# Alisah-Ozcan/HEonGPU

Hardware: AMD Instinct MI355X
Metric: homomorphic mults/sec (CKKS N=2^16, L=16) + NTT GB/s vs HBM roofline (higher is better)
Workload: dtype u64

## Files before the change

### heongpu_amd/__init__.py

```python
from . import _lib
from .api import (BFV, CKKS, SEC_NONE, SEC_128, SEC_192, SEC_256, TABLES_QP, TABLES_Q_BSK, OP_CKKS_RELIN, OP_CKKS_RESCALE,
                  OP_CKKS_GALOIS, OP_CKKS_ROTATE_HOISTED, OP_BFV_MULTIPLY, OP_BFV_RELIN, OP_BFV_GALOIS, E_INVALID, E_LOGIC, E_RUNTIME,
                  E_NODEVICE, Context, HEError, Rng, TfheContext, OP_KEYGEN_SECRET, OP_KEYGEN_PUBLIC,
                  OP_KEYGEN_SWITCH, OP_CKKS_ENCRYPT, OP_BFV_ENCRYPT, OP_BFV_DECRYPT, OP_BFV_DECODE, OP_CKKS_ENCODE,
                  OP_CKKS_DECODE, OP_BFV_MULTIPLY_PLAIN, OP_MPC_KEY_SHARE, OP_MPC_BFV_DECRYPT_MERGE, OP_MPC_REFRESH_SHARE, OP_MPC_REFRESH_MERGE,
                  MPC_PUBLIC_KEY,
                  MPC_GALOIS_KEY, MPC_RELIN_ROUND1, GATE_NAND, GATE_AND, GATE_AND_FIRST_NOT,
                  GATE_NOR, GATE_OR, GATE_XNOR, GATE_XOR, GATE_NOT, steps_to_galois_elt, linear_transform_plan, encoding_transform_factors, poly_eval_plan, eval_mod_plan, PolyEvalPlan, bootstrap_plan, BootstrapPlan, OP_CKKS_MOD_RAISE, OP_CKKS_BOOTSTRAP, MONOMIAL, CHEBYSHEV, POLY_POWER, POLY_LEAF, POLY_COMBINE, POLY_TAIL_NONE, POLY_TAIL_ONE, to_device, to_host, default_options, broadcast_key, broadcast_bytes, broadcast_path_name,
                  BCAST_FLAT, BCAST_TREE, BCAST_STAGED, BCAST_SAME_DEVICE, OP_CKKS_LOGIC_GATE, OP_BFV_LOGIC_GATE, LOGIC_AND,
                  LOGIC_OR, LOGIC_XOR, LOGIC_NAND, LOGIC_NOR, LOGIC_XNOR, LOGIC_NOT, GATE_B_NONE, GATE_B_CIPHER, GATE_B_PLAIN)

_lib.load()

__all__ = ["BFV", "CKKS", "SEC_NONE", "SEC_128", "SEC_192", "SEC_256", "TABLES_QP", "TABLES_Q_BSK", "Context", "HEError", "Rng",
           "steps_to_galois_elt", "linear_transform_plan", "encoding_transform_factors", "poly_eval_plan", "eval_mod_plan", "PolyEvalPlan", "bootstrap_plan", "BootstrapPlan", "MONOMIAL", "CHEBYSHEV", "POLY_POWER", "POLY_LEAF", "POLY_COMBINE", "POLY_TAIL_NONE", "POLY_TAIL_ONE", "to_device", "to_host", "default_options", "broadcast_key", "broadcast_bytes", "broadcast_path_name",
           "BCAST_FLAT", "BCAST_TREE", "BCAST_STAGED", "BCAST_SAME_DEVICE"]
```

### heongpu_amd/_lib.py

```python
import ctypes
import os

_HERE = os.path.dirname(os.path.abspath(__file__))
LIB_PATH = os.path.join(_HERE, "lib", "libhegpu.so")
if os.environ.get("HEGPU_AUDIT_LIB"):
    if os.path.basename(os.environ["HEGPU_AUDIT_LIB"]) != "libhegpu_audit.so":
        raise ImportError("HEGPU_AUDIT_LIB must name tests/audit/lib/libhegpu_audit.so")
    LIB_PATH = os.environ["HEGPU_AUDIT_LIB"]

u64 = ctypes.c_uint64
u64p = ctypes.c_void_p
c_int = ctypes.c_int
c_size_t = ctypes.c_size_t
voidp = ctypes.c_void_p



class LinearFactor(ctypes.Structure):
    _fields_ = [("diags", ctypes.c_void_p), ("n_diag", c_int), ("index", ctypes.POINTER(c_int)), ("n1", c_int), ("n2", c_int),
                ("baby_keys", ctypes.POINTER(ctypes.c_void_p)), ("baby_elts", ctypes.POINTER(c_int)),
                ("giant_keys", ctypes.POINTER(ctypes.c_void_p)), ("giant_elts", ctypes.POINTER(c_int))]


class PolyStep(ctypes.Structure):
    _fields_ = [("kind", ctypes.c_int32), ("dst", ctypes.c_int32), ("a", ctypes.c_int32), ("b", ctypes.c_int32),
                ("c", ctypes.c_int32), ("level", ctypes.c_int32), ("mul_level", ctypes.c_int32),
                ("rescale_first", ctypes.c_int32), ("rescale_after", ctypes.c_int32), ("n_terms", ctypes.c_int32),
                ("term_reg", ctypes.c_int32 * 15), ("scale", ctypes.c_double), ("tail_const", ctypes.c_double),
                ("w0", ctypes.c_double * 2), ("w", (ctypes.c_double * 2) * 15)]


class BootstrapConfig(ctypes.Structure):
    _fields_ = [("scale", ctypes.c_double), ("message_ratio", ctypes.c_double), ("K", ctypes.c_int32),
                ("sine_degree", ctypes.c_int32), ("double_angle", ctypes.c_int32), ("cts_level", ctypes.c_int32),
                ("cts_pieces", ctypes.c_int32), ("eval_level", ctypes.c_int32), ("stc_level", ctypes.c_int32),
                ("stc_pieces", ctypes.c_int32)]


class BootstrapPlan(ctypes.Structure):
    _fields_ = [("k1", ctypes.c_uint64), ("cts_level", ctypes.c_int32), ("cts_pieces", ctypes.c_int32),
                ("eval_level", ctypes.c_int32), ("stc_level", ctypes.c_int32), ("stc_pieces", ctypes.c_int32),
                ("out_level", ctypes.c_int32), ("K", ctypes.c_int32), ("sine_degree", ctypes.c_int32),
                ("double_angle", ctypes.c_int32), ("reserved", ctypes.c_int32), ("raise_scale", ctypes.c_double),
                ("cts_scale", ctypes.c_double * 5), ("cts_label", ctypes.c_double * 5), ("eval_in_scale", ctypes.c_double),
                ("eval_target_scale", ctypes.c_double), ("eval_out_scale", ctypes.c_double), ("stc_in_scale", ctypes.c_double),
                ("stc_scale", ctypes.c_double * 5), ("stc_label", ctypes.c_double * 5), ("out_scale", ctypes.c_double)]


SIGNATURES = [
    ("hegpu_last_error", ctypes.c_char_p, []),
    ("hegpu_version", ctypes.c_char_p, []),
    ("hegpu_context_create", c_int,
     [c_int, c_int, ctypes.POINTER(c_int), c_int, ctypes.POINTER(c_int), c_int, u64, c_int,
      ctypes.POINTER(voidp)]),
    ("hegpu_context_create_default", c_int, [c_int, c_int, c_int, u64, c_int, ctypes.POINTER(voidp)]),
    ("hegpu_context_create_from_primes", c_int,
     [c_int, c_int, ctypes.POINTER(u64), c_int, c_int, u64, ctypes.POINTER(voidp)]),
    ("hegpu_validate_coeff_modulus_values", c_int, [c_int, ctypes.POINTER(u64), c_int, c_int, c_int]),
    ("hegpu_context_destroy", None, [voidp]),
    ("hegpu_context_upload", c_int, [voidp]),
    ("hegpu_context_clone", c_int, [voidp, ctypes.POINTER(voidp)]),
    ("hegpu_context_upload_device", c_int, [voidp, c_int]),
    ("hegpu_context_device", c_int, [voidp]),
    ("hegpu_broadcast_key", c_int, [ctypes.POINTER(voidp), c_int, ctypes.POINTER(voidp), c_size_t, ctypes.POINTER(voidp)]),
    ("hegpu_broadcast_bytes", c_int, [ctypes.POINTER(c_int), c_int, ctypes.POINTER(voidp), c_size_t, ctypes.POINTER(voidp),
                                      ctypes.POINTER(c_int)]),
    ("hegpu_last_broadcast_path", c_int, []),
    ("hegpu_context_set_option", c_int, [voidp, ctypes.c_char_p, c_int]),
    ("hegpu_context_get_option", c_int, [voidp, ctypes.c_char_p, ctypes.POINTER(c_int)]),
    ("hegpu_tfhe_context_set_option", c_int, [voidp, ctypes.c_char_p, c_int]),
    ("hegpu_context_int", ctypes.c_long, [voidp, ctypes.c_char_p]),
    ("hegpu_context_get", ctypes.c_long, [voidp, ctypes.c_char_p, voidp, ctypes.c_long]),
    ("hegpu_context_device_ptr", voidp, [voidp, ctypes.c_char_p]),
    ("hegpu_steps_to_galois_elt", c_int, [c_int, c_int, c_int]),
    ("hegpu_ntt", c_int, [voidp, c_int, u64p, u64p, c_int, c_int, c_int, c_int, voidp, voidp, voidp]),
    ("hegpu_GPU_NTT", c_int, [voidp, c_int, u64p, u64p, c_int, c_int, c_int, voidp]),
    ("hegpu_GPU_NTT_Inplace", c_int, [voidp, c_int, u64p, c_int, c_int, c_int, voidp]),
    ("hegpu_GPU_INTT", c_int, [voidp, c_int, u64p, u64p, c_int, c_int, c_int, voidp]),
    ("hegpu_GPU_INTT_Inplace", c_int, [voidp, c_int, u64p, c_int, c_int, c_int, voidp]),
    ("hegpu_GPU_NTT_Modulus_Ordered_Inplace", c_int, [voidp, c_int, u64p, c_int, c_int, c_int, c_int, voidp, voidp]),
    ("hegpu_GPU_NTT_Poly_Ordered_Inplace", c_int, [voidp, c_int, u64p, c_int, c_int, c_int, c_int, voidp, voidp]),
    ("hegpu_addition", c_int, [voidp, u64p, u64p, u64p, c_int, c_int, c_int, c_int, voidp]),
    ("hegpu_cross_multiplication", c_int,
     [voidp, c_int, u64p, u64, u64p, u64, u64p, u64, c_int, c_int, voidp]),
    ("hegpu_cipher_broadcast", c_int, [voidp, u64p, u64, u64p, u64, c_int, c_int, c_int, c_int, c_int, voidp]),
    ("hegpu_mod_raise", c_int, [voidp, u64p, u64, u64p, u64, c_int, c_int, c_int, voidp]),
    ("hegpu_ckks_mod_raise", c_int, [voidp, u64p, u64, u64p, u64, c_int, c_int, voidp, c_size_t, voidp]),
    ("hegpu_keyswitch_multiply_accumulate", c_int,
     [voidp, u64p, u64, u64p, u64p, u64, c_int, c_int, c_int, c_int, c_int, c_int, voidp]),
    ("hegpu_base_conversion_DtoQtilde", c_int, [voidp, u64p, u64, u64p, u64, c_int, c_int, voidp]),
    ("hegpu_divide_round_lastq", c_int, [voidp, u64p, u64, u64p, u64, u64p, u64, c_int, c_int, voidp]),
    ("hegpu_divide_round_lastq_permute", c_int,
     [voidp, u64p, u64, u64p, u64, u64p, u64, c_int, c_int, c_int, voidp]),
    ("hegpu_divide_round_lastq_leveled_stage_one", c_int, [voidp, u64p, u64, u64p, u64, c_int, c_int, c_int, voidp]),
    ("hegpu_divide_round_lastq_leveled_stage_two", c_int,
     [voidp, u64p, u64, u64p, u64, u64p, u64, u64p, u64, c_int, c_int, c_int, voidp]),
    ("hegpu_move_cipher_leveled", c_int, [voidp, u64p, u64, u64p, u64, c_int, c_int, voidp]),
    ("hegpu_divide_round_lastq_rescale", c_int, [voidp, u64p, u64, u64p, u64, u64p, u64, c_int, c_int, voidp]),
    ("hegpu_divide_round_lastq_extended", c_int,
     [voidp, u64p, u64, u64p, u64, u64p, u64, c_int, c_int, c_int, voidp]),
    ("hegpu_fast_convertion", c_int, [voidp, u64p, u64, u64p, u64, u64p, u64, c_int, voidp]),
    ("hegpu_fast_floor", c_int, [voidp, u64p, u64, u64p, u64, c_int, voidp]),
    ("hegpu_workspace_bytes", c_size_t, [voidp, c_int, c_int, c_int]),
    ("hegpu_ckks_multiply", c_int, [voidp, u64p, u64, u64p, u64, u64p, u64, c_int, c_int, voidp]),
    ("hegpu_ckks_relinearize_inplace", c_int, [voidp, u64p, u64, u64p, c_int, c_int, voidp, c_size_t, voidp]),
    ("hegpu_probe_ckks_relinearize", c_int,
     [voidp, u64p, u64, u64p, c_int, c_int, voidp, c_size_t, ctypes.c_uint, voidp]),
    ("hegpu_ckks_rescale_inplace", c_int, [voidp, u64p, u64, c_int, c_int, voidp, c_size_t, voidp]),
    ("hegpu_ckks_apply_galois", c_int,
     [voidp, u64p, u64, u64p, u64, u64p, c_int, c_int, c_int, voidp, c_size_t, voidp]),
    ("hegpu_ckks_rotate_hoisted", c_int,
     [voidp, u64p, u64, u64p, u64, ctypes.POINTER(ctypes.c_void_p), ctypes.POINTER(c_int), c_int, c_int, c_int, voidp,
      c_size_t, voidp]),
    ("hegpu_ckks_diag_mac", c_int,
     [voidp, u64p, u64, c_int, u64p, c_int, ctypes.POINTER(c_int), c_int, u64p, u64, c_int, c_int, voidp]),
    ("hegpu_ckks_linear_transform_workspace_bytes", c_size_t, [voidp, c_int, c_int, c_int, c_int]),
    ("hegpu_ckks_linear_transform", c_int,
     [voidp, u64p, u64, u64p, u64, u64p, c_int, ctypes.POINTER(c_int), c_int, c_int, ctypes.POINTER(ctypes.c_void_p),
      ctypes.POINTER(c_int), ctypes.POINTER(ctypes.c_void_p), ctypes.POINTER(c_int), c_int, c_int, voidp, c_size_t, voidp]),
    ("hegpu_encoding_transform_shape", c_int,
     [c_int, c_int, c_int, ctypes.POINTER(c_int), ctypes.POINTER(c_int), ctypes.POINTER(c_int)]),
    ("hegpu_encoding_transform_fill", c_int, [c_int, c_int, c_int, c_int, c_int, ctypes.POINTER(c_int), voidp]),
    ("hegpu_poly_eval_plan_size", c_int,
     [c_int, voidp, c_int, c_int, c_int, c_int, ctypes.c_double, ctypes.c_double, ctypes.POINTER(u64), c_int,
      ctypes.POINTER(c_int)]),
    ("hegpu_poly_eval_plan_fill", c_int,
     [c_int, voidp, c_int, c_int, c_int, c_int, ctypes.c_double, ctypes.c_double, ctypes.POINTER(u64), c_int,
      ctypes.POINTER(PolyStep), c_int]),
    ("hegpu_eval_mod_plan_size", c_int,
     [c_int, c_int, c_int, c_int, ctypes.c_double, ctypes.c_double, ctypes.POINTER(u64), c_int, ctypes.POINTER(c_int)]),
    ("hegpu_eval_mod_plan_fill", c_int,
     [c_int, c_int, c_int, c_int, ctypes.c_double, ctypes.c_double, ctypes.POINTER(u64), c_int, ctypes.POINTER(PolyStep),
      c_int]),
    ("hegpu_ckks_weighted_sum", c_int,
     [voidp, ctypes.POINTER(ctypes.c_void_p), ctypes.POINTER(u64), ctypes.POINTER(c_int), ctypes.POINTER(ctypes.c_double),
      c_int, ctypes.c_double, ctypes.c_double, u64p, u64, c_int, c_int, voidp]),
    ("hegpu_ckks_double_sub", c_int,
     [voidp, u64p, u64, c_int, u64p, u64, c_int, ctypes.c_double, u64p, u64, c_int, c_int, voidp]),
    ("hegpu_ckks_poly_eval_workspace_bytes", c_size_t, [voidp, ctypes.POINTER(PolyStep), c_int, c_int, c_int]),
    ("hegpu_ckks_poly_eval", c_int,
     [voidp, u64p, u64, u64p, u64, ctypes.POINTER(PolyStep), c_int, u64p, c_int, c_int, voidp, c_size_t, voidp]),
    ("hegpu_ckks_conj_split", c_int, [voidp, u64p, u64, u64p, u64, u64p, u64p, u64, c_int, c_int, c_int, voidp]),
    ("hegpu_ckks_conj_merge", c_int, [voidp, u64p, u64, u64p, u64, u64p, u64, c_int, c_int, c_int, voidp]),
    ("hegpu_ckks_encoding_transform_workspace_bytes", c_size_t, [voidp, ctypes.POINTER(LinearFactor), c_int, c_int, c_int]),
    ("hegpu_ckks_coeff_to_slot", c_int,
     [voidp, u64p, u64, u64p, u64p, u64, ctypes.POINTER(LinearFactor), c_int, u64p, c_int, c_int, voidp, c_size_t, voidp]),
    ("hegpu_ckks_slot_to_coeff", c_int,
     [voidp, u64p, u64, u64p, u64, u64p, u64, ctypes.POINTER(LinearFactor), c_int, c_int, c_int, voidp, c_size_t, voidp]),
    ("hegpu_bootstrap_plan_fill", c_int,
     [ctypes.POINTER(BootstrapConfig), ctypes.POINTER(u64), c_int, ctypes.POINTER(BootstrapPlan)]),
    ("hegpu_ckks_bootstrap_workspace_bytes", c_size_t,
     [voidp, ctypes.POINTER(BootstrapPlan), ctypes.POINTER(PolyStep), c_int, ctypes.POINTER(LinearFactor), c_int,
      ctypes.POINTER(LinearFactor), c_int, c_int, c_int]),
    ("hegpu_ckks_bootstrap", c_int,
     [voidp, u64p, u64, u64p, u64, ctypes.POINTER(BootstrapPlan), ctypes.POINTER(PolyStep), c_int,
      ctypes.POINTER(LinearFactor), c_int, ctypes.POINTER(LinearFactor), c_int, u64p, u64p, u64p, u64p, c_int, voidp,
      c_size_t, voidp]),
    ("hegpu_ckks_gate_combine", c_int,
     [voidp, c_int, u64p, u64, c_int, u64p, c_int, u64, c_int, u64p, u64, c_int, ctypes.c_double, u64p, u64, c_int, c_int,
      voidp]),
    ("hegpu_bfv_gate_combine", c_int, [voidp, c_int, u64p, u64, u64p, c_int, u64, u64p, u64, u64p, u64, c_int, voidp]),
    ("hegpu_ckks_logic_gate", c_int,
     [voidp, c_int, u64p, u64, u64p, c_int, u64, u64p, ctypes.c_double, u64p, u64, c_int, c_int, voidp, c_size_t, voidp]),
    ("hegpu_bfv_logic_gate", c_int,
     [voidp, c_int, u64p, u64, u64p, c_int, u64, u64p, u64p, u64, c_int, voidp, c_size_t, voidp]),
    ("hegpu_bfv_multiply", c_int, [voidp, u64p, u64, u64p, u64, u64p, u64, c_int, voidp, c_size_t, voidp]),
    ("hegpu_bfv_relinearize_inplace", c_int, [voidp, u64p, u64, u64p, c_int, voidp, c_size_t, voidp]),
    ("hegpu_bfv_apply_galois", c_int,
     [voidp, u64p, u64, u64p, u64, u64p, c_int, c_int, voidp, c_size_t, voidp]),
    ("hegpu_rng_create", c_int, [u64, ctypes.POINTER(voidp)]),
    ("hegpu_rng_create_seeded", c_int, [ctypes.c_char_p, ctypes.POINTER(voidp)]),
    ("hegpu_rng_create_from_entropy", c_int, [ctypes.POINTER(voidp)]),
    ("hegpu_drbg_block", c_int, [ctypes.c_char_p, u64, u64, ctypes.POINTER(ctypes.c_uint32)]),
    ("hegpu_rng_destroy", None, [voidp]),
    ("hegpu_generate_secret_key", c_int, [voidp, voidp, c_int, u64p, voidp, c_size_t, voidp]),
    ("hegpu_generate_public_key", c_int, [voidp, voidp, u64p, u64p, voidp, c_size_t, voidp]),
    ("hegpu_generate_relin_key", c_int, [voidp, voidp, u64p, u64p, voidp, c_size_t, voidp]),
    ("hegpu_generate_switch_key", c_int, [voidp, voidp, u64p, u64p, u64p, voidp, c_size_t, voidp]),
    ("hegpu_generate_galois_key", c_int, [voidp, voidp, u64p, c_int, u64p, voidp, c_size_t, voidp]),
    ("hegpu_ckks_encrypt", c_int, [voidp, voidp, u64p, u64p, u64p, voidp, c_size_t, voidp]),
    ("hegpu_ckks_decrypt", c_int, [voidp, u64p, u64p, c_int, u64p, voidp]),
    ("hegpu_bfv_encrypt", c_int, [voidp, voidp, u64p, u64p, u64p, voidp, c_size_t, voidp]),
    ("hegpu_bfv_decrypt", c_int, [voidp, u64p, u64p, u64p, voidp, c_size_t, voidp]),
    ("hegpu_mpc_public_key_share", c_int, [voidp, voidp, voidp, u64p, u64p, voidp, c_size_t, voidp]),
    ("hegpu_mpc_relin_key_share_round1", c_int, [voidp, voidp, voidp, u64p, u64p, u64p, voidp, c_size_t, voidp]),
    ("hegpu_mpc_relin_key_share_round2", c_int, [voidp, voidp, u64p, u64p, u64p, u64p, voidp, c_size_t, voidp]),
    ("hegpu_mpc_galois_key_share", c_int, [voidp, voidp, voidp, u64p, c_int, u64p, voidp, c_size_t, voidp]),
    ("hegpu_mpc_accumulate", c_int, [voidp, ctypes.POINTER(ctypes.c_void_p), c_int, c_int, u64p, voidp]),
    ("hegpu_mpc_relin_key_finish", c_int, [voidp, ctypes.POINTER(ctypes.c_void_p), c_int, u64p, u64p, voidp]),
    ("hegpu_mpc_ckks_decrypt_share", c_int, [voidp, voidp, u64p, u64, u64p, c_int, u64p, c_int, voidp]),
    ("hegpu_mpc_ckks_decrypt_merge", c_int,
     [voidp, u64p, u64, ctypes.POINTER(ctypes.c_void_p), c_int, c_int, u64p, c_int, voidp]),
    ("hegpu_mpc_bfv_decrypt_share", c_int, [voidp, voidp, u64p, u64, u64p, u64p, c_int, voidp]),
    ("hegpu_mpc_bfv_decrypt_merge", c_int,
     [voidp, u64p, u64, ctypes.POINTER(ctypes.c_void_p), c_int, u64p, c_int, voidp, c_size_t, voidp]),
    ("hegpu_mpc_ckks_refresh_share", c_int,
     [voidp, voidp, voidp, u64p, u64, u64p, c_int, c_int, u64p, c_int, voidp, c_size_t, voidp]),
    ("hegpu_mpc_ckks_refresh_merge", c_int,
     [voidp, voidp, u64p, u64, ctypes.POINTER(ctypes.c_void_p), c_int, c_int, u64p, u64, c_int, voidp, c_size_t, voidp]),
    ("hegpu_mpc_bfv_refresh_share", c_int, [voidp, voidp, voidp, u64p, u64, u64p, u64p, c_int, voidp, c_size_t, voidp]),
    ("hegpu_mpc_bfv_refresh_merge", c_int,
     [voidp, voidp, u64p, u64, ctypes.POINTER(ctypes.c_void_p), c_int, u64p, u64, c_int, voidp, c_size_t, voidp]),
    ("hegpu_bfv_noise_rns", c_int, [voidp, u64p, u64p, u64p, voidp]),
    ("hegpu_bfv_plain_to_ntt", c_int, [voidp, u64p, u64p, voidp]),
    ("hegpu_negacyclic_shift", c_int, [voidp, u64p, u64p, c_int, c_int, c_int, voidp]),
    ("hegpu_ckks_constant_op", c_int, [voidp, c_int, u64p, ctypes.c_double, u64p, c_int, c_int, voidp]),
    ("hegpu_ckks_gaussian_integer_op", c_int,
     [voidp, c_int, u64p, ctypes.c_double, ctypes.c_double, u64p, c_int, c_int, voidp]),
    ("hegpu_ckks_mult_i", c_int, [voidp, u64p, u64p, c_int, c_int, c_int, voidp]),
    ("hegpu_cipherplain_multiplication", c_int, [voidp, u64p, u64p, u64p, c_int, voidp]),
    ("hegpu_bfv_plain_addsub", c_int, [voidp, u64p, u64p, u64p, c_int, voidp]),
    ("hegpu_bfv_multiply_plain", c_int, [voidp, u64p, u64p, u64p, voidp, c_size_t, voidp]),
    ("hegpu_bfv_encode", c_int, [voidp, voidp, c_int, u64p, voidp]),
    ("hegpu_ckks_encode", c_int, [voidp, voidp, c_int, ctypes.c_double, u64p, voidp, c_size_t, voidp]),
    ("hegpu_ckks_decode", c_int, [voidp, u64p, c_int, ctypes.c_double, voidp, voidp, c_size_t, voidp]),
    ("hegpu_ckks_encode_complex", c_int, [voidp, voidp, c_int, ctypes.c_double, u64p, voidp, c_size_t, voidp]),
    ("hegpu_ckks_decode_complex", c_int, [voidp, u64p, c_int, ctypes.c_double, voidp, voidp, c_size_t, voidp]),
    ("hegpu_ckks_encode_coeff", c_int, [voidp, voidp, c_int, ctypes.c_double, u64p, voidp]),
    ("hegpu_ckks_decode_coeff", c_int, [voidp, u64p, c_int, ctypes.c_double, voidp, voidp, c_size_t, voidp]),
    ("hegpu_ckks_encode_scalar", c_int, [voidp, ctypes.c_double, ctypes.c_double, u64p, voidp]),
    ("hegpu_bfv_decode", c_int, [voidp, u64p, u64p, voidp, c_size_t, voidp]),
    ("hegpu_tfhe_context_create", c_int, [ctypes.POINTER(voidp)]),
    ("hegpu_tfhe_context_destroy", None, [voidp]),
    ("hegpu_tfhe_context_int", ctypes.c_long, [voidp, ctypes.c_char_p]),
    ("hegpu_tfhe_prime", u64, [voidp]),
    ("hegpu_tfhe_prepare_bootkey", c_int, [voidp, u64p, u64p, voidp]),
    ("hegpu_tfhe_prepared_format", c_int, [voidp, u64p, c_int]),
    ("hegpu_tfhe_gate_precompute", c_int, [voidp, c_int, voidp, voidp, voidp, voidp, voidp, voidp, c_int, voidp]),
    ("hegpu_tfhe_bootstrapping", c_int, [voidp, voidp, voidp, u64p, voidp, voidp, c_int, voidp]),
    ("hegpu_tfhe_status", c_int, [voidp, voidp]),
    ("hegpu_tfhe_key_switching", c_int, [voidp, voidp, voidp, voidp, voidp, voidp, voidp, c_int, voidp]),
    ("hegpu_tfhe_generate_secret_key", c_int, [voidp, voidp, voidp, voidp, voidp]),
    ("hegpu_tfhe_generate_bootstrapping_key", c_int,
     [voidp, voidp, voidp, voidp, u64p, voidp, voidp, voidp, c_size_t, voidp]),
    ("hegpu_tfhe_encrypt", c_int, [voidp, voidp, voidp, voidp, c_int, voidp, voidp, voidp]),
    ("hegpu_tfhe_decrypt_phase", c_int, [voidp, voidp, voidp, voidp, c_int, voidp, voidp]),
    ("hegpu_tfhe_mux", c_int,
     [voidp, voidp, voidp, voidp, voidp, voidp, voidp, voidp, voidp, u64p, voidp, voidp, c_int, voidp, c_size_t,
      voidp]),
    ("hegpu_tfhe_gate", c_int,
     [voidp, c_int, voidp, voidp, voidp, voidp, voidp, voidp, u64p, voidp, voidp, c_int, voidp, c_size_t, voidp]),
]

_lib = None


def load():
    global _lib
    if _lib is not None:
        return _lib
    if not os.path.exists(LIB_PATH):
        raise ImportError(
            f"{LIB_PATH} not found: build it with `python -c 'import __graft_entry__ as g; g.build()'` "
            "or `make -C heongpu_amd/csrc`.  There is no CPU fallback.")
    import torch
    lib = ctypes.CDLL(LIB_PATH)
    for name, restype, argtypes in SIGNATURES:
        fn = getattr(lib, name)
        fn.restype = restype
        fn.argtypes = argtypes
# ... 3 lines not shown
```

### heongpu_amd/api.py

```python
import collections
import contextlib
import ctypes

import numpy as np

from . import _lib

BFV, CKKS = 1, 2
SEC_NONE, SEC_128, SEC_192, SEC_256 = 0, 128, 192, 256
TABLES_QP, TABLES_Q_BSK = 0, 1
OP_CKKS_RELIN, OP_CKKS_RESCALE, OP_CKKS_GALOIS, OP_BFV_MULTIPLY, OP_BFV_RELIN, OP_BFV_GALOIS = 1, 2, 3, 4, 5, 6
OP_CKKS_ROTATE_HOISTED = 17
OP_KEYGEN_SECRET, OP_KEYGEN_PUBLIC, OP_KEYGEN_SWITCH, OP_CKKS_ENCRYPT, OP_BFV_ENCRYPT, OP_BFV_DECRYPT, OP_BFV_DECODE = 7, 8, 9, 10, 11, 12, 13
OP_CKKS_ENCODE, OP_CKKS_DECODE = 14, 15
OP_BFV_MULTIPLY_PLAIN = 16
OP_MPC_KEY_SHARE, OP_MPC_BFV_DECRYPT_MERGE = 18, 19
OP_MPC_REFRESH_SHARE, OP_MPC_REFRESH_MERGE = 20, 21
MPC_PUBLIC_KEY, MPC_GALOIS_KEY, MPC_RELIN_ROUND1 = 0, 1, 2
TABLES_PLAIN = 2
OP_CKKS_LOGIC_GATE, OP_BFV_LOGIC_GATE = 22, 23
OP_CKKS_MOD_RAISE = 25
OP_CKKS_BOOTSTRAP = 26
LOGIC_AND, LOGIC_OR, LOGIC_XOR, LOGIC_NAND, LOGIC_NOR, LOGIC_XNOR, LOGIC_NOT = range(7)
GATE_B_NONE, GATE_B_CIPHER, GATE_B_PLAIN = 0, 1, 2
# ... 901 lines not shown

    def generate_secret_key(self, rng, stream=None):
        import torch
        lwe = torch.empty(self.int("n"), dtype=torch.int32, device="cuda")
        tlwe = torch.empty(self.int("N") * self.int("k"), dtype=torch.int32, device="cuda")
        _check(self._lib.hegpu_tfhe_generate_secret_key(self._h, rng._h, _ptr(lwe), _ptr(tlwe),
                                                        stream if stream is not None else _stream()))
        return lwe, tlwe

    def generate_bootstrapping_key(self, rng, lwe, tlwe, stream=None):
        import torch
        bk = torch.empty(self.int("bootkey_elems"), dtype=torch.int64, device="cuda")
        ks_a = torch.empty(self.int("kskey_a_elems"), dtype=torch.int32, device="cuda")
        ks_b = torch.empty(self.int("kskey_b_elems"), dtype=torch.int32, device="cuda")
        ws = torch.empty(self.int("N"), dtype=torch.int64, device="cuda")
        _check(self._lib.hegpu_tfhe_generate_bootstrapping_key(self._h, rng._h, _ptr(lwe), _ptr(tlwe), _ptr(bk),
                                                               _ptr(ks_a), _ptr(ks_b), _ptr(ws), ws.numel() * 8,
                                                               stream if stream is not None else _stream()))
        return bk, ks_a, ks_b

    def encrypt(self, rng, lwe, messages, stream=None):
        import torch
        shape = messages.numel()
        a = torch.empty(shape * self.int("n"), dtype=torch.int32, device="cuda")
        b = torch.empty(shape, dtype=torch.int32, device="cuda")
        _check(self._lib.hegpu_tfhe_encrypt(self._h, rng._h, _ptr(lwe), _ptr(messages), shape, _ptr(a), _ptr(b),
                                            stream if stream is not None else _stream()))
        return a, b

    def decrypt_phase(self, lwe, a, b, stream=None):
        import torch
        out = torch.empty(b.numel(), dtype=torch.int32, device="cuda")
        _check(self._lib.hegpu_tfhe_decrypt_phase(self._h, _ptr(lwe), _ptr(a), _ptr(b), b.numel(), _ptr(out),
                                                  stream if stream is not None else _stream()))
        return out

    def mux(self, a1, b1, a2, b2, ca, cb, out_a, out_b, prepared_bk, ks_a, ks_b, shape, ws, stream=None):
        _check(self._lib.hegpu_tfhe_mux(self._h, _ptr(a1), _ptr(b1), _ptr(a2), _ptr(b2), _ptr(ca), _ptr(cb),
                                        _ptr(out_a), _ptr(out_b), _ptr(prepared_bk), _ptr(ks_a), _ptr(ks_b), shape,
                                        _ptr(ws), ws.numel() * ws.element_size(),
                                        stream if stream is not None else _stream()))

    def gate(self, gate, a1, b1, a2, b2, out_a, out_b, prepared_bk, ks_a, ks_b, shape, ws, stream=None):
        _check(self._lib.hegpu_tfhe_gate(self._h, gate, _ptr(a1), _ptr(b1), _ptr(a2), _ptr(b2), _ptr(out_a),
                                         _ptr(out_b), _ptr(prepared_bk), _ptr(ks_a), _ptr(ks_b), shape, _ptr(ws),
                                         ws.numel() * ws.element_size(),
                                         stream if stream is not None else _stream()))


LinearTransformPlan = collections.namedtuple("LinearTransformPlan",
                                             "n1 n2 index baby_shifts giant_shifts pre_rotation")


def linear_transform_plan(diag_indices, slots, n1=None, stride=1):
    ks = sorted({int(k) % slots for k in diag_indices})
    if not ks:
        raise ValueError("a linear transform needs at least one diagonal")
    if stride < 1 or any(k % stride for k in ks):
        raise ValueError("every diagonal index is a multiple of the stride")
    if n1 is None:
        root = len(ks) ** 0.5
        n1 = min((1, 2, 4, 8, 16), key=lambda p: (abs(p - root), -p))
    if not 1 <= n1 <= 16:
        raise ValueError("the baby-step period lies in [1, 16]")
    qs = [k // stride for k in ks]
    baby = sorted({q % n1 for q in qs})
    giant = sorted({q // n1 for q in qs})
    if len(giant) > 16:
        raise ValueError(f"{len(giant)} giant steps, at most 16 fit one transform: choose a larger period")
    index = [[-1] * len(baby) for _ in giant]
    for pos, q in enumerate(qs):
        index[giant.index(q // n1)][baby.index(q % n1)] = pos
    return LinearTransformPlan(len(baby), len(giant), index, [stride * i for i in baby], [stride * j * n1 for j in giant],
                               [-stride * (q // n1) * n1 for q in qs])


EncodingTransformPiece = collections.namedtuple("EncodingTransformPiece", "stride stages offsets diagonals")


def encoding_transform_factors(n, inverse, pieces):
    import numpy as np
    lib = _lib.load()
    strides, stages, counts = ((ctypes.c_int * pieces)() for _ in range(3))
    _check(lib.hegpu_encoding_transform_shape(n, int(bool(inverse)), pieces, strides, stages, counts))
    out = []
    for p in range(pieces):
        offsets = (ctypes.c_int * counts[p])()
        values = np.empty((counts[p], n // 2), dtype=np.complex128)
        _check(lib.hegpu_encoding_transform_fill(n, int(bool(inverse)), pieces, p, counts[p], offsets,
                                                 values.ctypes.data))
        out.append(EncodingTransformPiece(strides[p], stages[p], list(offsets), values))
    return out


MONOMIAL, CHEBYSHEV = 0, 1
POLY_POWER, POLY_LEAF, POLY_COMBINE = 0, 1, 2
POLY_TAIL_NONE, POLY_TAIL_ONE = -1, -2
PolyEvalPlan = collections.namedtuple("PolyEvalPlan", "steps level scale out_limbs")


def poly_eval_plan(basis, coeffs, level, scale, target_scale, primes, max_deg=None, lead=True):
    lib = _lib.load()
    c = np.ascontiguousarray(np.asarray(coeffs, dtype=np.complex128).reshape(-1))
    pr = [int(p) for p in primes]
    arr = (ctypes.c_uint64 * max(len(pr), 1))(*pr)
    md = len(c) - 1 if max_deg is None else int(max_deg)
    args = (int(basis), c.ctypes.data, len(c), md, int(bool(lead)), int(level), float(scale), float(target_scale), arr,
            len(pr))
    count = ctypes.c_int(0)
    _check(lib.hegpu_poly_eval_plan_size(*args, ctypes.byref(count)))
    steps = (_lib.PolyStep * count.value)()
    _check(lib.hegpu_poly_eval_plan_fill(*args, steps, count.value))
    last = steps[count.value - 1]
    return PolyEvalPlan(steps, last.level, last.scale, last.level + 1 + last.rescale_after)


def eval_mod_plan(K, degree, double_angle, level, scale, target_scale, primes):
    lib = _lib.load()
    pr = [int(p) for p in primes]
    arr = (ctypes.c_uint64 * max(len(pr), 1))(*pr)
    args = (int(K), int(degree), int(double_angle), int(level), float(scale), float(target_scale), arr, len(pr))
    count = ctypes.c_int(0)
    _check(lib.hegpu_eval_mod_plan_size(*args, ctypes.byref(count)))
    steps = (_lib.PolyStep * count.value)()
    _check(lib.hegpu_eval_mod_plan_fill(*args, steps, count.value))
    last = steps[count.value - 1]
    return PolyEvalPlan(steps, last.level, last.scale, last.level + 1 + last.rescale_after)


class BootstrapPlan:

    def __init__(self, c, eval_mod):
        self.c, self.eval_mod = c, eval_mod
        for name, _t in c._fields_:
            setattr(self, name, getattr(c, name))
        self.k1 = int(c.k1)
        self.cts_scale, self.cts_label = list(c.cts_scale)[:c.cts_pieces], list(c.cts_label)[:c.cts_pieces]
        self.stc_scale, self.stc_label = list(c.stc_scale)[:c.stc_pieces], list(c.stc_label)[:c.stc_pieces]


def bootstrap_plan(primes, scale, cts_level, cts_pieces=3, stc_pieces=3, message_ratio=256.0, K=16, sine_degree=30,
                   double_angle=3, eval_level=-1, stc_level=-1):
    lib = _lib.load()
    pr = [int(p) for p in primes]
    arr = (ctypes.c_uint64 * max(len(pr), 1))(*pr)
    cfg = _lib.BootstrapConfig(float(scale), float(message_ratio), int(K), int(sine_degree), int(double_angle), int(cts_level),
                               int(cts_pieces), int(eval_level), int(stc_level), int(stc_pieces))
    c = _lib.BootstrapPlan()
    _check(lib.hegpu_bootstrap_plan_fill(ctypes.byref(cfg), arr, len(pr), ctypes.byref(c)))
    return BootstrapPlan(c, eval_mod_plan(c.K, c.sine_degree, c.double_angle, c.eval_level, c.eval_in_scale,
                                          c.eval_target_scale, pr))


def steps_to_galois_elt(steps, n, group_order):
    return int(_lib.load().hegpu_steps_to_galois_elt(steps, n, group_order))
```

### heongpu_amd/csrc/cabi.cpp

```cpp
#include "../../include/hegpu.h"
#include "../../include/hegpu_bench.h"
#include "context.hpp"
#include "encoding_transform.hpp"
#include "host_params.hpp"
#include "poly_eval.hpp"
#include "ops.hpp"
#include <cmath>
#include <complex>
#include <cstddef>
#include "tfhe.hpp"
#include <algorithm>
#include <cerrno>
#include <climits>
#include <mutex>
#include <unordered_map>
#include <vector>
#include <cstring>
#include <sys/random.h>
#include <memory>
#include <new>
#include <stdexcept>
#include <string>

#ifdef HEGPU_FP_AUDIT_HEADER
// ... 710 lines not shown
    return hip_ret(rns_moddown_permute((const u64*) in, in_stride, (const u64*) in2, in2_stride, (u64*) out,
                                       out_stride, c.moddown(depth), galois_elt, batch, (hipStream_t) stream),
                   "hegpu_divide_round_lastq_permute");
}

#define SEAM_CKKS(ctx, depth, batch, min_limbs)                                                                    \
    NEED_CTX(ctx);                                                                                                 \
    const Context& c = (ctx)->c;                                                                                   \
    if (c.scheme != SCHEME_CKKS) return fail(HEGPU_E_INVALID, "CKKS context required");                            \
    if ((depth) < 0 || c.Q_size - (depth) < (min_limbs)) return fail(HEGPU_E_INVALID, "invalid depth");            \
    if ((batch) < 0) return fail(HEGPU_E_INVALID, "batch must not be negative");                                   \
    if ((batch) == 0) return 0;                                                                                    \
    const int l = c.Q_size - (depth);                                                                              \
    (void) l

int hegpu_divide_round_lastq_leveled_stage_one(hegpu_context* ctx, const uint64_t* in, uint64_t in_stride, uint64_t* out,
                                               uint64_t out_stride, int rescale, int depth, int batch,
                                               hegpu_stream stream)
{
    SEAM_CKKS(ctx, depth, batch, rescale ? 2 : 1);
    if (!rescale && c.P_size != 1) return fail(HEGPU_E_LOGIC, "the leveled stages serve a single special prime (method I)");
    return hip_ret(rns_moddown_stage_one((const u64*) in, in_stride, (u64*) out, out_stride, c.moddown(depth, rescale != 0),
                                         batch, (hipStream_t) stream),
                   "hegpu_divide_round_lastq_leveled_stage_one");
}

int hegpu_divide_round_lastq_leveled_stage_two(hegpu_context* ctx, const uint64_t* in_last, uint64_t last_stride,
                                               const uint64_t* in, uint64_t in_stride, const uint64_t* ct,
                                               uint64_t ct_stride, uint64_t* out, uint64_t out_stride, int switchkey,
                                               int depth, int batch, hegpu_stream stream)
{
    SEAM_CKKS(ctx, depth, batch, 1);
    if (c.P_size != 1) return fail(HEGPU_E_LOGIC, "the leveled stages serve a single special prime (method I)");
    if (!ct) return fail(HEGPU_E_INVALID, "ct must not be NULL");
    return hip_ret(rns_moddown_stage_two((const u64*) in_last, last_stride, (const u64*) in, in_stride, (const u64*) ct,
                                         ct_stride, (u64*) out, out_stride, c.moddown(depth), switchkey ? 2 : 1, batch,
                                         (hipStream_t) stream),
                   "hegpu_divide_round_lastq_leveled_stage_two");
}

int hegpu_move_cipher_leveled(hegpu_context* ctx, const uint64_t* in, uint64_t in_stride, uint64_t* out,
                              uint64_t out_stride, int depth, int batch, hegpu_stream stream)
{
    SEAM_CKKS(ctx, depth, batch, 2);
    return hip_ret(rns_copy_limbs((const u64*) in, (u64) l * c.n, in_stride, (u64*) out, (u64) l * c.n, out_stride,
                                  c.n_power, l - 1, 2, batch, (hipStream_t) stream),
                   "hegpu_move_cipher_leveled");
}

int hegpu_divide_round_lastq_rescale(hegpu_context* ctx, const uint64_t* in_last, uint64_t last_stride,
                                     const uint64_t* in, uint64_t in_stride, uint64_t* out, uint64_t out_stride,
                                     int depth, int batch, hegpu_stream stream)
{
    SEAM_CKKS(ctx, depth, batch, 2);
    return hip_ret(rns_moddown_stage_two((const u64*) in_last, last_stride, (const u64*) in, in_stride, nullptr, 0,
                                         (u64*) out, out_stride, c.moddown(depth, true), 0, batch, (hipStream_t) stream),
                   "hegpu_divide_round_lastq_rescale");
}

int hegpu_divide_round_lastq_extended(hegpu_context* ctx, const uint64_t* in, uint64_t in_stride, const uint64_t* ct,
                                      uint64_t ct_stride, uint64_t* out, uint64_t out_stride, int mode, int depth,
                                      int batch, hegpu_stream stream)
{
    NEED_CTX(ctx);
    const Context& c = ctx->c;
    if (mode < 0 || mode > 2) return fail(HEGPU_E_INVALID, "mode must be 0, 1 or 2");
    if (c.scheme == SCHEME_BFV && depth != 0) return fail(HEGPU_E_INVALID, "BFV ciphertexts have no depth");
    if (depth < 0 || depth >= c.Q_size) return fail(HEGPU_E_INVALID, "invalid depth");
    if (mode && !ct) return fail(HEGPU_E_INVALID, "ct must not be NULL");
    if (batch < 0) return fail(HEGPU_E_INVALID, "batch must not be negative");
    if (batch == 0) return 0;
    return hip_ret(rns_moddown_extended((const u64*) in, in_stride, (const u64*) ct, ct_stride, (u64*) out, out_stride,
                                        c.moddown(depth), mode, batch, (hipStream_t) stream),
                   "hegpu_divide_round_lastq_extended");
}

int hegpu_fast_convertion(hegpu_context* ctx, const uint64_t* in1, uint64_t s1, const uint64_t* in2, uint64_t s2,
                          uint64_t* out, uint64_t so, int batch, hegpu_stream stream)
{
    NEED_CTX(ctx);
    const Context& c = ctx->c;
    if (c.scheme != SCHEME_BFV) return fail(HEGPU_E_INVALID, "BFV context required");
    return hip_ret(rns_fast_convertion((const u64*) in1, s1, (const u64*) in2, s2, (u64*) out, so, c.behz,
                                       c.n_power, batch, (hipStream_t) stream),
                   "hegpu_fast_convertion");
}

int hegpu_fast_floor(hegpu_context* ctx, const uint64_t* in, uint64_t si, uint64_t* out, uint64_t so, int batch,
                     hegpu_stream stream)
{
    NEED_CTX(ctx);
    const Context& c = ctx->c;
    if (c.scheme != SCHEME_BFV) return fail(HEGPU_E_INVALID, "BFV context required");
    return hip_ret(rns_fast_floor((const u64*) in, si, (u64*) out, so, c.behz, c.n_power, batch,
                                  (hipStream_t) stream),
                   "hegpu_fast_floor");
}

#define SAME_OP(name) static_assert((int) HEGPU_OP_##name == (int) OP_##name, "HEGPU_OP_" #name " != OP_" #name)
SAME_OP(CKKS_RELIN); SAME_OP(CKKS_RESCALE); SAME_OP(CKKS_GALOIS); SAME_OP(BFV_MULTIPLY); SAME_OP(BFV_RELIN);
SAME_OP(BFV_GALOIS); SAME_OP(KEYGEN_SECRET); SAME_OP(KEYGEN_PUBLIC); SAME_OP(KEYGEN_SWITCH); SAME_OP(CKKS_ENCRYPT);
SAME_OP(BFV_ENCRYPT); SAME_OP(BFV_DECRYPT); SAME_OP(BFV_DECODE); SAME_OP(CKKS_ENCODE); SAME_OP(CKKS_DECODE);
SAME_OP(BFV_MULTIPLY_PLAIN); SAME_OP(CKKS_ROTATE_HOISTED); SAME_OP(MPC_KEY_SHARE); SAME_OP(MPC_BFV_DECRYPT_MERGE);
SAME_OP(MPC_REFRESH_SHARE); SAME_OP(MPC_REFRESH_MERGE); SAME_OP(CKKS_LOGIC_GATE); SAME_OP(BFV_LOGIC_GATE); SAME_OP(CKKS_MOD_RAISE);
SAME_OP(CKKS_BOOTSTRAP);
#undef SAME_OP

size_t hegpu_workspace_bytes(const hegpu_context* ctx, int op, int depth, int batch)
{
    if (!ctx || batch <= 0) return 0;
    return ops_workspace_elems(ctx->c, op, depth, batch) * sizeof(u64);
}

#define CHECK_OP(ctx, want_scheme, op, depth, batch, ws, ws_bytes)                                            \
    do {                                                                                                      \
        if ((ctx)->c.scheme != (want_scheme)) return fail(HEGPU_E_INVALID, "context scheme mismatch");        \
        if ((batch) < 0) return fail(HEGPU_E_INVALID, "batch must not be negative");                          \
        if ((batch) == 0) return 0;                                            \
        if ((depth) < 0 || (depth) >= (ctx)->c.Q_size) return fail(HEGPU_E_INVALID, "invalid depth");         \
        if ((op) && (!(ws) || (ws_bytes) < hegpu_workspace_bytes(ctx, op, depth, batch)))                     \
            return fail(HEGPU_E_INVALID, "workspace too small");                                              \
    } while (0)

int hegpu_ckks_multiply(hegpu_context* ctx, const uint64_t* ct1, uint64_t s1, const uint64_t* ct2, uint64_t s2,
                        uint64_t* out, uint64_t so, int depth, int batch, hegpu_stream stream)
{
    NEED_CTX(ctx);
    if (ctx->c.scheme != SCHEME_CKKS) return fail(HEGPU_E_INVALID, "context scheme mismatch");
    if (depth < 0 || depth >= ctx->c.Q_size) return fail(HEGPU_E_INVALID, "invalid depth");
    return hip_ret(op_ckks_multiply(ctx->c, (const u64*) ct1, s1, (const u64*) ct2, s2, (u64*) out, so, depth, batch,
                                    (hipStream_t) stream),
                   "hegpu_ckks_multiply");
}

int hegpu_ckks_relinearize_inplace(hegpu_context* ctx, uint64_t* ct, uint64_t cs, const uint64_t* key, int depth,
                                   int batch, void* ws, size_t ws_bytes, hegpu_stream stream)
{
    NEED_CTX(ctx);
    CHECK_OP(ctx, SCHEME_CKKS, OP_CKKS_RELIN, depth, batch, ws, ws_bytes);
    return hip_ret(op_ckks_relinearize(ctx->c, (u64*) ct, cs, (const u64*) key, depth, batch, (u64*) ws,
                                       (hipStream_t) stream),
                   "hegpu_ckks_relinearize_inplace");
}

int hegpu_probe_ckks_relinearize(hegpu_context* ctx, uint64_t* ct, uint64_t cs, const uint64_t* key, int depth,
                                 int batch, void* ws, size_t ws_bytes, unsigned phases, hegpu_stream stream)
{
    NEED_CTX(ctx);
    CHECK_OP(ctx, SCHEME_CKKS, OP_CKKS_RELIN, depth, batch, ws, ws_bytes);
    if (ctx->c.P_size != 1) return fail(HEGPU_E_LOGIC, "the phase probe covers key-switching method I");
    return hip_ret(op_ckks_relinearize(ctx->c, (u64*) ct, cs, (const u64*) key, depth, batch, (u64*) ws,
                                       (hipStream_t) stream, phases),
                   "hegpu_probe_ckks_relinearize");
}

int hegpu_ckks_rescale_inplace(hegpu_context* ctx, uint64_t* ct, uint64_t cs, int depth, int batch, void* ws,
                               size_t ws_bytes, hegpu_stream stream)
{
    NEED_CTX(ctx);
    CHECK_OP(ctx, SCHEME_CKKS, OP_CKKS_RESCALE, depth, batch, ws, ws_bytes);
    if (depth >= ctx->c.Q_size - 1) return fail(HEGPU_E_LOGIC, "no modulus left to rescale by");
    return hip_ret(op_ckks_rescale(ctx->c, (u64*) ct, cs, depth, batch, (u64*) ws, (hipStream_t) stream),
                   "hegpu_ckks_rescale_inplace");
}

static bool spans_overlap(const uint64_t* a, uint64_t a_stride, uint64_t a_item, const uint64_t* b, uint64_t b_stride,
                          uint64_t b_item, int batch)
{
    if (batch <= 0) return false;
    const __int128 W = sizeof(uint64_t);
    const __int128 a0 = (__int128) (uintptr_t) a, b0 = (__int128) (uintptr_t) b;
    const __int128 ai = (__int128) a_item * W, bi = (__int128) b_item * W;
    auto hit = [&](__int128 pa, __int128 pb) { return pa < pb + bi && pb < pa + ai; };
    if (batch == 1) return hit(a0, b0);
    {
        const __int128 a1 = a0 + ((__int128) (batch - 1) * a_stride + a_item) * W;
        const __int128 b1 = b0 + ((__int128) (batch - 1) * b_stride + b_item) * W;
        if (!(a0 < b1 && b0 < a1)) return false;
    }
    if (a_stride == b_stride) {
        const __int128 st = (__int128) a_stride * W;
        for (long k = -(long) (batch - 1); k <= (long) (batch - 1); k++)
            if (hit(a0, b0 + k * st)) return true;
        return false;
    }
    if (batch <= 1024) {
        for (int i = 0; i < batch; i++)
            for (int j = 0; j < batch; j++)
                if (hit(a0 + (__int128) i * a_stride * W, b0 + (__int128) j * b_stride * W)) return true;
        return false;
    }
    return true;
}

int hegpu_ckks_apply_galois(hegpu_context* ctx, const uint64_t* ct, uint64_t cs, uint64_t* out, uint64_t so,
                            const uint64_t* key, int galois_elt, int depth, int batch, void* ws, size_t ws_bytes,
                            hegpu_stream stream)
{
    NEED_CTX(ctx);
    CHECK_OP(ctx, SCHEME_CKKS, OP_CKKS_GALOIS, depth, batch, ws, ws_bytes);
    {
        const uint64_t words = (uint64_t) 2 * (ctx->c.Q_size - depth) * ctx->c.n;
        if (spans_overlap(ct, cs, words, out, so, words, batch))
            return fail(HEGPU_E_INVALID, "apply_galois: out must not alias ct (the result buffer must not contain the input)");
    }
    if (galois_elt <= 0 || !(galois_elt & 1) || galois_elt >= 2 * (int) ctx->c.n)
        return fail(HEGPU_E_INVALID, "apply_galois: Galois elements are odd and below 2N");
    return hip_ret(op_ckks_apply_galois(ctx->c, (const u64*) ct, cs, (u64*) out, so, (const u64*) key, galois_elt, depth,
                                        batch, (u64*) ws, (hipStream_t) stream),
                   "hegpu_ckks_apply_galois");
}

int hegpu_mod_raise(hegpu_context* ctx, const uint64_t* in, uint64_t in_stride, uint64_t* out, uint64_t out_stride,
                    int limbs, int parts, int batch, hegpu_stream stream)
{
    if (!ctx) return fail(HEGPU_E_INVALID, "null context");
    if (!in || !out) return fail(HEGPU_E_INVALID, "mod_raise: null argument");
    if (batch < 1 || batch > 65535) return fail(HEGPU_E_INVALID, "mod_raise: 1 to 65535 items per call");
    if (parts < 1 || parts > 3) return fail(HEGPU_E_INVALID, "mod_raise: parts is 1, 2 or 3");
    if (limbs < 1 || limbs > ctx->c.Q_size) return fail(HEGPU_E_INVALID, "mod_raise: 1 <= limbs <= Q");
    if (spans_overlap(in, in_stride, (uint64_t) parts * ctx->c.n, out, out_stride, (uint64_t) parts * limbs * ctx->c.n, batch))
        return fail(HEGPU_E_INVALID, "mod_raise: out must not overlap in");
    NEED_CTX(ctx);
    const Context& c = ctx->c;
    return hip_ret(rns_mod_raise((const u64*) in, in_stride, (u64*) out, out_stride, c.plan_qp.mods, c.n_power, limbs, parts,
                                 batch, (hipStream_t) stream),
                   "hegpu_mod_raise");
}

int hegpu_ckks_mod_raise(hegpu_context* ctx, const uint64_t* ct, uint64_t cs, uint64_t* out, uint64_t so, int out_depth,
                         int batch, void* ws, size_t ws_bytes, hegpu_stream stream)
{
    if (!ctx) return fail(HEGPU_E_INVALID, "null context");
    if (ctx->c.scheme != SCHEME_CKKS) return fail(HEGPU_E_INVALID, "context scheme mismatch");
    if (!ct || !out || !ws) return fail(HEGPU_E_INVALID, "ckks_mod_raise: null argument");
    if (batch < 1) return fail(HEGPU_E_INVALID, "ckks_mod_raise: batch must be at least 1");
    if (out_depth < 0 || out_depth >= ctx->c.Q_size) return fail(HEGPU_E_INVALID, "ckks_mod_raise: 0 <= out_depth < Q");
    const uint64_t in_words = (uint64_t) 2 * ctx->c.n, out_words = in_words * (ctx->c.Q_size - out_depth);
    const size_t need = ops_workspace_elems(ctx->c, OP_CKKS_MOD_RAISE, out_depth, batch) * sizeof(u64);
    if (ws_bytes < need) return fail(HEGPU_E_INVALID, "workspace too small");
    if (spans_overlap(ct, cs, in_words, out, so, out_words, batch))
        return fail(HEGPU_E_INVALID, "ckks_mod_raise: out must not overlap ct");
    if (spans_overlap((const uint64_t*) ws, 0, need / sizeof(u64), out, so, out_words, batch) ||
        spans_overlap((const uint64_t*) ws, 0, need / sizeof(u64), ct, cs, in_words, batch))
        return fail(HEGPU_E_INVALID, "ckks_mod_raise: the workspace must overlap neither out nor ct");
    NEED_CTX(ctx);
    return hip_ret(op_ckks_mod_raise(ctx->c, (const u64*) ct, cs, (u64*) out, so, out_depth, batch, (u64*) ws,
                                     (hipStream_t) stream),
                   "hegpu_ckks_mod_raise");
}

int hegpu_ckks_rotate_hoisted(hegpu_context* ctx, const uint64_t* ct, uint64_t cs, uint64_t* out, uint64_t so,
                              const uint64_t* const* keys, const int* galois_elts, int count, int depth, int batch,
                              void* ws, size_t ws_bytes, hegpu_stream stream)
{
    NEED_CTX(ctx);
    CHECK_OP(ctx, SCHEME_CKKS, OP_CKKS_GALOIS, depth, batch, ws, ws_bytes);
    if (count <= 0 || !keys || !galois_elts) return fail(HEGPU_E_INVALID, "rotate_hoisted: empty element list");
    const uint64_t words = (uint64_t) 2 * (ctx->c.Q_size - depth) * ctx->c.n;
    if (batch > 1 && so < (uint64_t) count * words) return fail(HEGPU_E_INVALID, "rotate_hoisted: out_stride too small");
    if (spans_overlap(ct, cs, words, out, so, (uint64_t) count * words, batch))
        return fail(HEGPU_E_INVALID, "rotate_hoisted: out must not alias ct (the result buffer must not contain the input)");
    for (int i = 0; i < count; i++) {
        if (galois_elts[i] == 0) continue;
        if (galois_elts[i] < 0 || !(galois_elts[i] & 1) || galois_elts[i] >= 2 * (int) ctx->c.n)
            return fail(HEGPU_E_INVALID, "rotate_hoisted: Galois elements are odd and below 2N");
        if (!keys[i]) return fail(HEGPU_E_INVALID, "rotate_hoisted: Galois key not present!");
    }
    const int group = (ctx->c.fused_moddown && ctx->c.ntt_galois)
                          ? ops_rotate_hoisted_accumulators(ctx->c, depth, batch, ws_bytes / sizeof(u64)) : 1;
    return hip_ret(op_ckks_rotate_hoisted(ctx->c, (const u64*) ct, cs, (u64*) out, so, (const u64* const*) keys,
                                          galois_elts, count, depth, batch, (u64*) ws, (hipStream_t) stream, group),
                   "hegpu_ckks_rotate_hoisted");
}

static bool diag_index_ok(const int* index, int n1, int n2, int n_diag)
{
    for (int k = 0; k < n1 * n2; k++)
        if (index[k] < -1 || index[k] >= n_diag) return false;
    return true;
}

int hegpu_ckks_diag_mac(hegpu_context* ctx, const uint64_t* rot, uint64_t rot_stride, int n1, const uint64_t* diags,
                        int n_diag, const int* index, int n2, uint64_t* out, uint64_t out_stride, int depth, int batch,
                        hegpu_stream stream)
{
    NEED_CTX(ctx);
    CHECK_OP(ctx, SCHEME_CKKS, 0, depth, batch, nullptr, 0);
    if (n1 < 1 || n1 > 16 || n2 < 1 || n2 > 16)
        return fail(HEGPU_E_INVALID, "diag_mac: n1 and n2 lie in [1, 16] (16 products per 128-bit sum, 256 indices by value)");
    if (!rot || !diags || !index || !out || n_diag < 1) return fail(HEGPU_E_INVALID, "diag_mac: null argument");
    if (!diag_index_ok(index, n1, n2, n_diag)) return fail(HEGPU_E_INVALID, "diag_mac: index outside [-1, n_diag)");
    if (batch > 65535) return fail(HEGPU_E_INVALID, "diag_mac: at most 65535 items per call");
    const uint64_t words = (uint64_t) 2 * (ctx->c.Q_size - depth) * ctx->c.n;
    if (spans_overlap(rot, rot_stride, (uint64_t) n1 * words, out, out_stride, (uint64_t) n2 * words, batch))
        return fail(HEGPU_E_INVALID, "diag_mac: out must not overlap rot");
    return hip_ret(rns_ckks_diag_mac((const u64*) rot, rot_stride, n1, (const u64*) diags, n_diag, index, n2, (u64*) out,
                                     out_stride, ctx->c.plan_qp.mods, ctx->c.n_power, ctx->c.Q_size - depth, batch,
                                     (hipStream_t) stream),
                   "hegpu_ckks_diag_mac");
}

size_t hegpu_ckks_linear_transform_workspace_bytes(const hegpu_context* ctx, int n1, int n2, int depth, int batch)
{
    if (!ctx || batch <= 0 || n1 < 1 || n1 > 16 || n2 < 1 || n2 > 16 || depth < 0 || depth >= ctx->c.Q_size) return 0;
    return ops_linear_transform_workspace_elems(ctx->c, n1, n2, depth, batch) * sizeof(u64);
// ... 1560 lines not shown
```

### heongpu_amd/csrc/context.cpp

```cpp
#include "context.hpp"
#include <cerrno>
#include <climits>
#include <cstdlib>
#include "host_params.hpp"
#include <algorithm>
#include <cmath>
#include <cstdlib>
#include <cstring>
#include <stdexcept>

namespace hegpu {

using host::inv_mod_prime;
using host::mul_mod;

typedef std::vector<u64> vec;

static void append(vec& dst, const vec& src) { dst.insert(dst.end(), src.begin(), src.end()); }

void Context::build_host()
{
    n = ((u64) 1) << n_power;
    Qp_size = Q_size + P_size;
    const int Q = Q_size, P = P_size, Qp = Qp_size;
// ... 542 lines not shown
                memcpy(&a, &vd, 8);
                memcpy(&b, &vi, 8);
                return make_ulonglong2(a, b);
            };
            hn[k] = pair(ninv[k]);
            hw[k] = pair(w1n);
        } else {
            hn[k] = make_ulonglong2(ninv[k], shoup_companion(ninv[k], q));
            hw[k] = make_ulonglong2(w1n, shoup_companion(w1n, q));
        }
    }
    p.count = cnt;
    p.has_fp = p.has_int = 0;
    for (int k = 0; k < cnt; k++) (hm[k].fp ? p.has_fp : p.has_int) = 1;
    p.fp.assign(cnt, 0);
    for (int k = 0; k < cnt; k++) p.fp[k] = hm[k].fp ? 1 : 0;
    p.bits.assign(cnt, 0);
    for (int k = 0; k < cnt; k++) p.bits[k] = (unsigned char) hm[k].bit;
    u64 qmax = 0;
    for (int k = 0; k < cnt; k++) qmax = mods[k] > qmax ? mods[k] : qmax;
    p.lazy_q_max = (~0ull - 2 * qmax) / (4ull * (u64) n_power);
    hipError_t e;
    if ((e = to_device(hm, &p.mods)) != hipSuccess) return e;
    if ((e = to_device(htw, &p.tw)) != hipSuccess) return e;
    if ((e = to_device(hitw, &p.itw)) != hipSuccess) return e;
    if ((e = to_device(htwB, &p.twB)) != hipSuccess) return e;
    if ((e = to_device(hitwB, &p.itwB)) != hipSuccess) return e;
    if ((e = to_device(htwB8, &p.twB8)) != hipSuccess) return e;
    if ((e = to_device(hn, &p.ninv)) != hipSuccess) return e;
    return to_device(hw, &p.w1ninv);
}

static void free_plan(NttPlan& p)
{
    if (p.mods) (void) hipFree(p.mods);
    if (p.tw) (void) hipFree(p.tw);
    if (p.itw) (void) hipFree(p.itw);
    if (p.twB) (void) hipFree(p.twB);
    if (p.itwB) (void) hipFree(p.itwB);
    if (p.twB8) (void) hipFree(p.twB8);
    if (p.ninv) (void) hipFree(p.ninv);
    if (p.w1ninv) (void) hipFree(p.w1ninv);
    p = NttPlan();
}

hipError_t Context::upload()
{
    if (uploaded) return hipSuccess;
    for (int k = 0; k < DRBG_GAUSS_MAX; k++)
        gauss_cdt.t[k] = (u64) (erf(((double) k + 0.5) / (3.2 * 1.4142135623730951)) * 9223372036854775808.0);
    hipError_t e = hipGetDevice(&device);
    if (e != hipSuccess) return e;
    if ((e = build_plan(plan_qp, host["modulus"], host["ntt_table"], host["intt_table"], host["n_inverse"],
                        n_power, fp_ntt)) != hipSuccess)
        return e;
    const struct { const char* name; const u64** slot; const int** ints; } rows[] = {
        {"psi_half", &tab.psi_half}, {"last_q_modinv", &tab.last_q_modinv}, {"half", &tab.half},
        {"half_mod", &tab.half_mod}, {"factor", &tab.factor},
        {"m2_md_W0", &tab.m2_md_W0}, {"m2_md_G", &tab.m2_md_G}, {"m2_md_C", &tab.m2_md_C},
        {"rescaled_last_q_modinv", &tab.rescaled_last_q_modinv}, {"rescaled_half_mod", &tab.rescaled_half_mod},
        {"rescaled_half", &tab.rescaled_half}, {"mod_raise_half_mod", &tab.mod_raise_half_mod},
        {"base_change_matrix_Bsk", &behz.base_change_matrix_Bsk},
        {"inv_punctured_prod_mod_base_array", &behz.inv_punctured_prod_mod_base_array},
        {"base_change_matrix_m_tilde", &behz.base_change_matrix_m_tilde},
        {"inv_m_tilde_mod_Bsk", &behz.inv_m_tilde_mod_Bsk}, {"prod_q_mod_Bsk", &behz.prod_q_mod_Bsk},
        {"inv_prod_q_mod_Bsk", &behz.inv_prod_q_mod_Bsk}, {"base_change_matrix_q", &behz.base_change_matrix_q},
        {"base_change_matrix_msk", &behz.base_change_matrix_msk},
        {"inv_punctured_prod_mod_B_array", &behz.inv_punctured_prod_mod_B_array},
        {"behz_mtilde_inv_punct", &behz.mtilde_inv_punct}, {"behz_t_inv_punct", &behz.t_inv_punct},
        {"behz_invq_inv_punct_B", &behz.invq_inv_punct_B}, {"behz_msk_mod_q", &behz.msk_mod_q},
        {"behz_fc_matrix", &behz.fc_matrix}, {"behz_fc_c1", &behz.fc_c1}, {"behz_ff_matrix", &behz.ff_matrix},
        {"behz_ff_tc", &behz.ff_tc}, {"behz_ff_q_matrix", &behz.ff_q_matrix},
        {"behz_ff_msk_matrix", &behz.ff_msk_matrix}, {"behz_ff_prod_B", &behz.ff_prod_B},
        {"behz_ff_neg_prod_B", &behz.ff_neg_prod_B}, {"prod_B_mod_q", &behz.prod_B_mod_q},
        {"Mi", &tab.Mi}, {"Mi_inv", &tab.Mi_inv}, {"upper_half_threshold", &tab.upper_half_threshold},
        {"decryption_modulus", &tab.decryption_modulus}, {"special_fft_roots_table", &tab.special_fft_roots_table},
        {"special_ifft_roots_table", &tab.special_ifft_roots_table},
        {"coeff_div_plain_modulus", &tab.coeff_div_plain_modulus}, {"upper_halfincrement", &tab.upper_halfincrement},
        {"Qi_t", &tab.Qi_t}, {"Qi_gamma", &tab.Qi_gamma}, {"Qi_inverse", &tab.Qi_inverse},
        {"m2_Mi_inv", &tab.m2_Mi_inv}, {"m2_matrix", &tab.m2_matrix}, {"m2_prod", &tab.m2_prod},
        {"m2_matrix_mg", &tab.m2_matrix_mg}, {"m2_negprod_mg", &tab.m2_negprod_mg},
        {"new_prime_locations", nullptr, &tab.new_prime_locations},
        {"new_input_locations", nullptr, &tab.new_input_locations}, {"m2_I_j", nullptr, &tab.m2_I_j},
        {"m2_I_location", nullptr, &tab.m2_I_location}, {"encoding_location", nullptr, &tab.encoding_location},
        {"reverse_order", nullptr, &tab.reverse_order}, {"mpc_refresh_order", nullptr, &tab.mpc_refresh_order},
    };
    for (const auto& r : rows) {
        auto it = host.find(r.name);
        if (it == host.end()) continue;
        if (r.slot) {
            u64* d = nullptr;
            if ((e = to_device(it->second, &d)) != hipSuccess) return e;
            dev[r.name] = d;
            *r.slot = d;
        } else {
            std::vector<int> v(it->second.begin(), it->second.end());
            int* d = nullptr;
            if ((e = to_device(v, &d)) != hipSuccess) return e;
            dev[r.name] = d;
            *r.ints = d;
        }
    }
    if (scheme == SCHEME_BFV) {
        if ((e = build_plan(plan_merge, host["q_Bsk_merge_modulus"], host["q_Bsk_merge_ntt_tables"],
                            host["q_Bsk_merge_intt_tables"], host["q_Bsk_n_inverse"], n_power, fp_ntt)) != hipSuccess)
            return e;
        if (host.count("plain_modulus2") &&
            (e = build_plan(plan_plain, host["plain_modulus2"], host["plain_ntt_tables"], host["plain_intt_tables"],
                            host["n_plain_inverse"], n_power, fp_ntt)) != hipSuccess)
            return e;
        behz.ibase = plan_merge.mods;
        behz.obase = plan_merge.mods + Q_size;
        behz.m_tilde = make_mod(((u64) 1) << 32);
        behz.plain = make_mod(plain_modulus);
        behz.inv_prod_q_mod_m_tilde = hv.inv_prod_q_mod_m_tilde;
        behz.inv_prod_B_mod_m_sk = hv.inv_prod_B_mod_m_sk;
        behz.ibase_size = Q_size;
        behz.obase_size = bsk_size;
        behz.split = behz_split;
    }
    uploaded = true;
    return hipDeviceSynchronize();
}

namespace {
struct OptDesc {
    enum Rule { PLAIN, NOT_1_OR_3, BEFORE_UPLOAD, MIRROR_BEHZ };
    const char* name;
    const char* env;
    int lo, hi;
    int ContextHost::*i;
    bool ContextHost::*b;
    Rule rule;
    constexpr OptDesc(const char* nm, const char* ev, int l, int h, int ContextHost::*m, Rule r = PLAIN)
        : name(nm), env(ev), lo(l), hi(h), i(m), b(nullptr), rule(r) {}
    constexpr OptDesc(const char* nm, const char* ev, bool ContextHost::*m, Rule r = PLAIN)
        : name(nm), env(ev), lo(0), hi(1), i(nullptr), b(m), rule(r) {}
};
typedef ContextHost H;
const OptDesc kOptions[] = {
    {"fused_row_mac", "HEGPU_FUSED_ROW_MAC", -1, 1, &H::fused_row_mac},
    {"fused_moddown", "HEGPU_FUSED_MODDOWN", &H::fused_moddown},
    {"col_multi", "HEGPU_COL_MULTI", -1, 1, &H::col_multi},
    {"single_pass", "HEGPU_SINGLE_PASS", -1, 1, &H::single_pass},
    {"ntt_galois", "HEGPU_NTT_GALOIS", &H::ntt_galois},
    {"galois_scatter", "HEGPU_GALOIS_SCATTER", &H::galois_scatter},
    {"fuse_inverse", "HEGPU_FUSE_INVERSE", &H::fuse_inverse},
    {"copy_along", "HEGPU_COPY_ALONG", &H::copy_along},
    {"digit_split", "HEGPU_DIGIT_SPLIT", -1, 4, &H::digit_split, OptDesc::NOT_1_OR_3},
    {"fp_ntt", "HEGPU_FP_NTT", &H::fp_ntt, OptDesc::BEFORE_UPLOAD},
    {"behz_split", "HEGPU_BEHZ_SPLIT", -1, 1, &H::behz_split, OptDesc::MIRROR_BEHZ},
    {"fused_tensor", "HEGPU_FUSED_TENSOR", &H::fused_tensor},
    {"moddown_in_mac", "HEGPU_MODDOWN_IN_MAC", &H::moddown_in_mac},
};
const OptDesc* find_option(const char* name)
{
    for (const OptDesc& o : kOptions)
        if (name && !strcmp(o.name, name)) return &o;
    return nullptr;
}
}

int Context::set_option(const char* name, int value)
{
    const OptDesc* d = find_option(name);
    if (!d) return 1;
    if (value < d->lo || value > d->hi || (d->rule == OptDesc::NOT_1_OR_3 && (value == 1 || value == 3))) return 2;
    if (d->rule == OptDesc::BEFORE_UPLOAD && uploaded) return 3;
    if (d->i) this->*d->i = value;
    else this->*d->b = value != 0;
    if (d->rule == OptDesc::MIRROR_BEHZ) behz.split = value;
    return 0;
}

int Context::get_option(const char* name, int* value) const
{
    const OptDesc* d = find_option(name);
    if (!d || !value) return 1;
    *value = d->i ? this->*d->i : (int) (this->*d->b);
    return 0;
}

bool env_long(const char* name, long* out)
{
    const char* e = getenv(name);
    if (!e || !*e) return false;
    char* end = nullptr;
    errno = 0;
    const long v = strtol(e, &end, 10);
    if (errno || end == e || *end) return false;
    *out = v;
    return true;
}

void Context::seed_options_from_env()
{
    for (const OptDesc& o : kOptions) {
        long v;
        if (env_long(o.env, &v) && v >= INT_MIN && v <= INT_MAX)
            (void) set_option(o.name, (int) v);
    }
}

void Context::release_device()
{
    free_plan(plan_qp);
    free_plan(plan_merge);
    free_plan(plan_plain);
    for (auto& kv : dev)
        if (kv.second) (void) hipFree(kv.second);
    dev.clear();
    uploaded = false;
}

Context::~Context()
{
    if (uploaded) release_device();
}

NttArgs Context::ntt_args(int table_set) const
{
    const NttPlan& p = table_set == 2 ? plan_plain : (table_set ? plan_merge : plan_qp);
    NttArgs a{};
    a.mods = p.mods;
    a.tw = p.tw;
    a.itw = p.itw;
    a.twB = p.twB;
    a.itwB = p.itwB;
    a.twB8 = p.twB8;
    a.ninv = p.ninv;
    a.w1ninv = p.w1ninv;
    a.n_power = n_power;
    a.mod_count = p.count;
    a.col_multi = col_multi;
    a.single_pass = single_pass;
    a.plan_has_fp = p.has_fp;
    a.plan_has_int = p.has_int;
    a.lazy_q_max = p.lazy_q_max;
    return a;
}

ModDown Context::moddown(int depth, bool rescale) const
{
    const int l = Q_size - depth;
    if (!rescale)
        return {plan_qp.mods, tab.half, tab.half_mod, tab.last_q_modinv, n_power, Qp_size - depth, l, Qp_size, Q_size,
                P_size};
    const int row = triangle_offset(Q_size - 1, depth);
    return {plan_qp.mods, tab.rescaled_half + depth, tab.rescaled_half_mod + row, tab.rescaled_last_q_modinv + row,
            n_power, l, l - 1, l, l - 1, 1};
}

}
```

### heongpu_amd/csrc/context.hpp

```cpp
#pragma once
#include "modarith.cuh"
#include "ntt.hpp"
#include "rns.hpp"
#include <map>
#include <string>
#include "drbg.hpp"
#include <vector>

namespace hegpu {

bool env_long(const char* name, long* out);


enum Scheme { SCHEME_BFV = 1, SCHEME_CKKS = 2 };

inline int triangle_offset(int first, int depth)
{
    int location = 0;
    for (int i = 0; i < depth; i++) location += first - i;
    return location;
}

struct NttPlan {
    Mod* mods = nullptr;
    ulonglong2* tw = nullptr;
    ulonglong2* itw = nullptr;
    ulonglong2* twB = nullptr;
    ulonglong2* itwB = nullptr;
    double* twB8 = nullptr;
    ulonglong2* ninv = nullptr;
    ulonglong2* w1ninv = nullptr;
    int count = 0;
    int has_fp = 0, has_int = 0;
    std::vector<unsigned char> fp;
    std::vector<unsigned char> bits;
    u64 lazy_q_max = 0;
};

struct DevTables {
    const u64 *psi_half, *last_q_modinv, *half, *half_mod, *factor;
    const u64 *m2_md_W0, *m2_md_G, *m2_md_C, *m2_Mi_inv, *m2_matrix, *m2_prod, *m2_matrix_mg, *m2_negprod_mg;
    const int *m2_I_j, *m2_I_location;
    const u64 *rescaled_last_q_modinv, *rescaled_half_mod, *rescaled_half;
    const u64* mod_raise_half_mod;
    const u64 *Mi, *Mi_inv, *upper_half_threshold, *decryption_modulus, *special_fft_roots_table, *special_ifft_roots_table;
    const int *new_prime_locations, *new_input_locations, *reverse_order, *mpc_refresh_order;
    const u64 *coeff_div_plain_modulus, *upper_halfincrement, *Qi_t, *Qi_gamma, *Qi_inverse;
    const int* encoding_location;
};

struct ContextHost {
    int scheme = 0;
    int n_power = 0;
    u64 n = 0;
    int Q_size = 0, P_size = 0, Qp_size = 0;
    int bsk_size = 0;
    u64 plain_modulus = 0;
    std::vector<u64> primes;
    std::map<std::string, std::vector<u64>> host;
    struct HostVals {
        u64 half = 0;
        std::vector<u64> rescaled_half;
        u64 mod_raise_half = 0;
        std::vector<u64> new_prime_locations;
        u64 Q_mod_t = 0, upper_threshold = 0, gamma = 0, mulq_inv_t = 0, mulq_inv_gamma = 0, inv_gamma = 0;
        u64 inv_prod_q_mod_m_tilde = 0, inv_prod_B_mod_m_sk = 0;
    } hv;
    struct M2Level {
        int d = 0, rc = 0;
        int off_digits = 0;
        int off_mi = 0;
        int off_matrix = 0;
        int off_prod = 0;
    };
    std::vector<M2Level> m2_levels;
    int m2_width = 0;
    int fused_row_mac = -1;
    bool fused_moddown = true;
    int col_multi = -1;
    int single_pass = -1;
    bool ntt_galois = true;
    bool galois_scatter = true;
    int digit_split = -1;
    bool copy_along = true;
    bool fuse_inverse = true;
    bool moddown_in_mac = true;
    bool fused_tensor = true;
    bool fp_ntt = true;
    int behz_split = -1;
};

struct Context : ContextHost {
    void seed_options_from_env();
    int set_option(const char* name, int value);
    int get_option(const char* name, int* value) const;
    GaussCdt gauss_cdt{};

    bool uploaded = false;
    int device = -1;
    NttPlan plan_qp;
    NttPlan plan_merge;
    NttPlan plan_plain;
    std::map<std::string, void*> dev;
    DevTables tab{};
    BehzDev behz{};

    ~Context();
    void build_host();
    hipError_t upload();
    void release_device();

    NttArgs ntt_args(int table_set) const;
    ModDown moddown(int depth, bool rescale = false) const;
};

}
```

### heongpu_amd/csrc/ntt.hip

```cpp
#include "ntt.hpp"
#define HEGPU_FP_TU ntt
#include "fpmod.cuh"

namespace hegpu {

#define NTT_THREADS 256

#ifdef NTT_ABLATION_HEADER
#include NTT_ABLATION_HEADER
#else
__device__ __forceinline__ u64 gld(const u64* p) { return *p; }
__device__ __forceinline__ void gst(u64* p, u64 v) { *p = v; }
#define NTT_ABLATE_BFLY(x, y, w)
#define NTT_ABLATE_FPBFLY(x, y, w)
#define NTT_ABLATE_TW(load, root0, s) (load)
#define NTT_FP_TW(t, i, c) ((t)[i])
#endif

__device__ __forceinline__ u64 csub(u64 x, u64 m) { return (x >= m) ? x - m : x; }

typedef unsigned long long u64x2_t __attribute__((ext_vector_type(2)));
struct ConstTw {
    const u64x2_t __attribute__((address_space(4)))* p;
    __device__ __forceinline__ ulonglong2 operator[](u32 i) const
    {
        const u64x2_t v = p[i];
        return make_ulonglong2(v.x, v.y);
    }
};
__device__ __forceinline__ ConstTw const_tw(const ulonglong2* t)
{
#pragma clang diagnostic push
#pragma clang diagnostic ignored "-Wold-style-cast"
    return ConstTw{(const u64x2_t __attribute__((address_space(4)))*) reinterpret_cast<const u64x2_t*>(t)};
#pragma clang diagnostic pop
}

__device__ __forceinline__ int ld_const_i32(const int* p)
{
#pragma clang diagnostic push
#pragma clang diagnostic ignored "-Wold-style-cast"
    return *(const int __attribute__((address_space(4)))*) p;
#pragma clang diagnostic pop
}
__device__ __forceinline__ Mod ld_const_mod(const Mod* p)
{
#pragma clang diagnostic push
#pragma clang diagnostic ignored "-Wold-style-cast"
    const u64 __attribute__((address_space(4)))* w = (const u64 __attribute__((address_space(4)))*) reinterpret_cast<const u64*>(p);
#pragma clang diagnostic pop
    static_assert(sizeof(Mod) == 56, "seven words");
    Mod m;
    m.q = w[0];
    m.mu = w[1];
    m.r_hi = w[2];
    m.r_lo = w[3];
    m.r64 = w[4];
    m.qinv = w[5];
    const u64 bf = w[6];
    m.bit = (u32) bf;
    m.fp = (u32) (bf >> 32);
    return m;
}

__device__ __forceinline__ void fp_ct_bfly(double& x, double& y, ulonglong2 w, const FC& c)
{
    NTT_ABLATE_FPBFLY(x, y, w);
    const double t = fp_mul(y, as_f64(w.x), as_f64(w.y), c);
    y = x - t;
    x = x + t;
    FP_AUDIT_VAL(c, FPM_SUM, x);
    FP_AUDIT_VAL(c, FPM_SUM, y);
}
__device__ __forceinline__ void fp_ct_bfly(double& x, double& y, double w, const FC& c)
{
    const double t = fp_mul_nc(y, w, c);
    y = x - t;
    x = x + t;
    FP_AUDIT_VAL(c, FPM_SUM, x);
    FP_AUDIT_VAL(c, FPM_SUM, y);
}
struct FpSched { unsigned before; bool at_end; };
#define FP_STAGE_GROW(b) (1.25 * (b) + 0.5)
#define FP_BOUND_LIMIT 7.9
#define FP_HANDOVER 0.51
#define FP_UNREDUCED_IN 1.05
constexpr FpSched fp_sched(int stages, double b_in, double b_out_max)
{
    unsigned m = 0;
    double b = b_in;
    for (int s = 0; s < stages; s++) {
        if (FP_STAGE_GROW(b) > FP_BOUND_LIMIT) {
            m |= 1u << s;
            b = 0.5;
        }
        b = FP_STAGE_GROW(b);
    }
    return FpSched{m, b > b_out_max};
}
template <int LOGR, typename TW>
__device__ __forceinline__ void fp_ct_radix(double (&x)[1 << LOGR], TW tw, u32 root0,
                                            const FC& c, unsigned before, bool at_end)
{
#pragma unroll
    for (int s = 0; s < LOGR; s++) {
        FP_STAGE(c, 31 - __builtin_clz(root0) + s);
        if ((before >> s) & 1u) {
#pragma unroll
            for (int k = 0; k < (1 << LOGR); k++) x[k] = fp_reduce(x[k], c);
        }
        const int half = (1 << LOGR) >> (s + 1);
#pragma unroll
        for (int b = 0; b < (1 << s); b++) {
            const ulonglong2 w = NTT_ABLATE_TW(NTT_FP_TW(tw, (root0 << s) + b, c), root0, s);
#pragma unroll
            for (int j = 0; j < half; j++) fp_ct_bfly(x[b * 2 * half + j], x[b * 2 * half + j + half], w, c);
        }
    }
    FP_STAGE(c, 31 - __builtin_clz(root0) + LOGR);
    if (at_end) {
#pragma unroll
        for (int k = 0; k < (1 << LOGR); k++) x[k] = fp_reduce(x[k], c);
    }
}
template <int S1> struct FpColSched {
    static constexpr FpSched s = fp_sched(S1, FP_UNREDUCED_IN, FP_HANDOVER);
    static constexpr unsigned a_before = s.before & ((1u << (S1 - 4)) - 1u);
    static constexpr unsigned b_before = (s.before >> (S1 - 4)) & 15u;
    static constexpr bool b_at_end = s.at_end;
};
__device__ __forceinline__ void fp_ct_radix16_tb(double (&x)[16], const ulonglong2* __restrict__ tb, const FC& c)
{
#pragma unroll
    for (int s = 0; s < 4; s++) {
        const int half = 8 >> s;
        if (s > 0) FP_STAGE(c, (c).stage + 1);
#pragma unroll
        for (int b = 0; b < (1 << s); b++) {
            const ulonglong2 w = NTT_ABLATE_TW(NTT_FP_TW(tb, ((1 << s) - 1 + b) * 16, c), (u32) b, s);
#pragma unroll
            for (int j = 0; j < half; j++) fp_ct_bfly(x[b * 2 * half + j], x[b * 2 * half + j + half], w, c);
        }
    }
    FP_STAGE(c, (c).stage + 1);
#pragma unroll
    for (int k = 0; k < 16; k++) x[k] = fp_canon(x[k], c);
}

__device__ __forceinline__ void fp_ct_radix16_tb8(double (&x)[16], const double* __restrict__ tb, const FC& c)
{
#pragma unroll
    for (int s = 0; s < 4; s++) {
        const int half = 8 >> s;
// ... 636 lines not shown
            } else {
#pragma unroll
                for (int k = 0; k < 16; k++) dy[k] = fp_reduce(fp_from_u64(dv[k]), fc);
            }
            if (a.half_on) {
                const double half_hm = fp_from_u64(a.half_mod[ps.mod]);
#pragma unroll
                for (int k = 0; k < 16; k++) dy[k] = fp_reduce(dy[k] - half_hm, fc);
            }
#pragma unroll
            for (int k = 0; k < 16; k++) FP_AUDIT_VAL(fc, FPM_SUM, dy[k]);
        } else {
            if (a.half_on) {
                const u64 half_hm = a.half_mod[ps.mod];
#pragma unroll
                for (int k = 0; k < 16; k++) dv[k] = sub_mod(reduce64(add_mod(dv[k], a.half, half_qP), md), half_hm, md.q);
            } else if (!LAZY && a.mods[ps.digit].q > 8 * md.q) {
#pragma unroll
                for (int k = 0; k < 16; k++) dv[k] = reduce64(dv[k], md);
            }
        }
    }
    if constexpr (FP) {
        double x[16];
        if constexpr (NSA > 0) {
#pragma unroll
            for (int gi = 0; gi < G; gi++) {
                const int L = tt + 256 * gi;
                const int c = L % CT, rb = L / CT;
                double y[RA];
#pragma unroll
                for (int k = 0; k < RA; k++) {
                    if constexpr (DECOMP) y[k] = dy[gi * RA + k];
                    else y[k] = fp_from_u64(gld(&src[(u64) (rb + 16 * k) * 256 + c]));
                }
                fp_ct_radix<NSA>(y, tw, 1u, fc, FpColSched<S1>::a_before, false);
#pragma unroll
                for (int k = 0; k < RA; k++) limb[single_pos<S1>(rb + 16 * k, g * CT + c)] = as_bits(y[k]);
            }
            __syncthreads();
#pragma unroll
            for (int k = 0; k < 16; k++) x[k] = as_f64(limb[single_pos<S1>(16 * r1 + k, g * CT + col)]);
        } else {
#pragma unroll
            for (int k = 0; k < 16; k++) {
                if constexpr (DECOMP) x[k] = dy[k];
                else x[k] = fp_from_u64(src[(u64) k * 256 + col]);
            }
        }
        fp_ct_radix<4>(x, tw, (u32) (RA + r1), fc, FpColSched<S1>::b_before, FpColSched<S1>::b_at_end);
#pragma unroll
        for (int k = 0; k < 16; k++) limb[single_pos<S1>(16 * r1 + k, g * CT + col)] = as_bits(x[k]);
    } else {
        u64 x[16];
        if constexpr (NSA > 0) {
#pragma unroll
            for (int gi = 0; gi < G; gi++) {
                const int L = tt + 256 * gi;
                const int c = L % CT, rb = L / CT;
                u64 y[RA];
#pragma unroll
                for (int k = 0; k < RA; k++) {
                    if constexpr (DECOMP) y[k] = dv[gi * RA + k];
                    else y[k] = gld(&src[(u64) (rb + 16 * k) * 256 + c]);
                }
                ct_radix<NSA, LAZY>(y, tw, 1u, qc);
#pragma unroll
                for (int k = 0; k < RA; k++) limb[single_pos<S1>(rb + 16 * k, g * CT + c)] = y[k];
            }
            __syncthreads();
#pragma unroll
            for (int k = 0; k < 16; k++) x[k] = limb[single_pos<S1>(16 * r1 + k, g * CT + col)];
        } else {
#pragma unroll
            for (int k = 0; k < 16; k++) {
                if constexpr (DECOMP) x[k] = dv[k];
                else x[k] = src[(u64) k * 256 + col];
            }
        }
        ct_radix<4, LAZY>(x, tw, (u32) (RA + r1), qc);
#pragma unroll
        for (int k = 0; k < 16; k++) limb[single_pos<S1>(16 * r1 + k, g * CT + col)] = x[k];
    }
    __syncthreads();
    u64* lds = limb + g * 4096;
    const int row = tt >> 4, i0 = tt & 15;
    const u32 crow = g * 16 + row;
    const ulonglong2* __restrict__ tb = a.twB + ((u64) ps.mod * (15u << (a.n_power - 4))) + ((u64) crow * 15 * 16 + i0);
    u64 r[16];
    if constexpr (FP) {
        double x[16];
#pragma unroll
        for (int k = 0; k < 16; k++) x[k] = as_f64(lds[row_phys(row * 256 + i0 + 16 * k)]);
        fp_ct_radix<4>(x, tw, (1u << S1) + crow, fc, 0u, true);
#pragma unroll
        for (int k = 0; k < 16; k++) lds[row_phys(row * 256 + i0 + 16 * k)] = as_bits(x[k]);
        wave_lds_fence();
#pragma unroll
        for (int k = 0; k < 8; k++) {
            ulonglong2 v = *reinterpret_cast<const ulonglong2*>(&lds[row_phys(row * 256 + 16 * i0 + 2 * k)]);
            x[2 * k] = as_f64(v.x);
            x[2 * k + 1] = as_f64(v.y);
        }
        fp_ct_radix16_tb8(x, a.twB8 + ((u64) ps.mod * (15u << (a.n_power - 4))) + ((u64) crow * 15 * 16 + i0), fc);
#pragma unroll
        for (int k = 0; k < 16; k++) r[k] = fp_to_u64(x[k]);
    } else {
        u64 x[16];
#pragma unroll
        for (int k = 0; k < 16; k++) x[k] = lds[row_phys(row * 256 + i0 + 16 * k)];
        ct_radix<4, LAZY>(x, tw, (1u << S1) + crow, qc);
#pragma unroll
        for (int k = 0; k < 16; k++) lds[row_phys(row * 256 + i0 + 16 * k)] = x[k];
        wave_lds_fence();
#pragma unroll
        for (int k = 0; k < 8; k++) {
            ulonglong2 v = *reinterpret_cast<const ulonglong2*>(&lds[row_phys(row * 256 + 16 * i0 + 2 * k)]);
            x[2 * k] = v.x;
            x[2 * k + 1] = v.y;
        }
        ct_radix16_tb<LAZY>(x, tb, qc);
        if (LAZY) {
#pragma unroll
            for (int k = 0; k < 16; k++) r[k] = reduce64(x[k], md);
        } else {
#pragma unroll
            for (int k = 0; k < 16; k++) r[k] = csub(csub(csub(x[k], qc.q4), 2 * qc.q), qc.q);
        }
    }
    wave_lds_fence();
#pragma unroll
    for (int k = 0; k < 8; k++)
        *reinterpret_cast<ulonglong2*>(&lds[row_phys(row * 256 + 16 * i0 + 2 * k)]) = make_ulonglong2(r[2 * k], r[2 * k + 1]);
    wave_lds_fence();
    row_store_all(a, ps, md, a.out + ps.out_off, (u64) g * 4096 + row * 256 + i0, lds, row, i0);
}

template <int S1, bool DECOMP = false>
__global__ __launch_bounds__(16 << S1, 4) void ntt_fwd_single(NttArgs a)
{
    extern __shared__ __attribute__((aligned(16))) u64 limb[];
    const PolySel ps = select_poly(a, blockIdx.x);
    if (DECOMP && a.skip_identity && ps.mod == ps.digit) return;
    const Mod md = a.mods[ps.mod];
    if (md.fp) fwd_single_body<S1, true, false, DECOMP>(a, ps, md, limb);
    else if (fwd_stages_lazy(md, a.lazy_q_max)) fwd_single_body<S1, false, true, DECOMP>(a, ps, md, limb);
    else fwd_single_body<S1, false, false, DECOMP>(a, ps, md, limb);
}

static_assert(ks_unreduced_exit(16, 60) == 16 && ks_unreduced_exit(17, 60) == 12 && ks_unreduced_exit(21, 60) == 12, "");
static_assert(ks_unreduced_exit(22, 60) == 8 && ks_unreduced_exit(32, 60) == 8 && ks_unreduced_exit(33, 60) == 0, "");
static_assert(ks_unreduced_exit(4, 61) == 16 && ks_unreduced_exit(8, 61) == 8 && ks_unreduced_exit(9, 61) == 0, "");

template <bool LAZY, int ROOM = 8, int EXIT = 0>
__device__ __forceinline__ void ks_row_digit(u64 (&x)[16], const u64* __restrict__ p, u64* lds,
                                             const ulonglong2* twa, const ulonglong2* __restrict__ tb,
                                             const QC& qc, const Mod& md, int row, int i0)
{
    static_assert(EXIT == 0 || (!LAZY && (EXIT == 8 || ((EXIT == 12 || EXIT == 16) && ROOM == 16))), "exit bound");
    constexpr CsSched CS = cs_sched(8, ROOM, EXIT ? EXIT : 8);
#pragma unroll
    for (int k = 0; k < 16; k++) x[k] = gld(&p[row * 256 + i0 + 16 * k]);
#pragma unroll
    for (int s = 0; s < 4; s++) {
        const int half = 8 >> s;
        const int cs = LAZY ? 0 : (int) (((CS.c8 >> s) & 1u) * 2u + ((CS.c4 >> s) & 1u));
#pragma unroll
        for (int b = 0; b < (1 << s); b++) {
            const ulonglong2 w = twa[((1 << s) - 1 + b) * 16 + row];
#pragma unroll
            for (int j = 0; j < half; j++) ct_bfly_cs(x[b * 2 * half + j], x[b * 2 * half + j + half], w, qc, cs);
        }
    }
#pragma unroll
    for (int k = 0; k < 16; k++) lds[row_phys(row * 256 + i0 + 16 * k)] = x[k];
    wave_lds_fence();
#pragma unroll
    for (int k = 0; k < 8; k++) {
        ulonglong2 v = *reinterpret_cast<const ulonglong2*>(&lds[row_phys(row * 256 + 16 * i0 + 2 * k)]);
        x[2 * k] = v.x;
        x[2 * k + 1] = v.y;
    }
    ct_radix16_tb<LAZY, (CS.c8 >> 4), (CS.c4 >> 4)>(x, tb, qc);
    if (!LAZY && EXIT == 0) {
#pragma unroll
        for (int k = 0; k < 16; k++) x[k] = csub(csub(csub(x[k], qc.q4), 2 * qc.q), qc.q);
    }
    wave_lds_fence();
#pragma unroll
    for (int k = 0; k < 8; k++)
        *reinterpret_cast<ulonglong2*>(&lds[row_phys(row * 256 + 16 * i0 + 2 * k)]) =
            make_ulonglong2(x[2 * k], x[2 * k + 1]);
    wave_lds_fence();
#pragma unroll
    for (int k = 0; k < 16; k++) x[k] = lds[row_phys(row * 256 + i0 + 16 * k)];
    wave_lds_fence();
}

struct KsIdx { int item, tile, slot; bool valid; int d0, d1; };
__host__ __device__ __forceinline__ unsigned ks_slots(const KsMacArgs& a, int kind)
{
    const int all = a.slot_count ? a.slot_count : a.rc;
    if (a.int_slot_count <= 0 || kind == 0) return (unsigned) all;
    return kind == 1 ? (unsigned) a.int_slot_count : (unsigned) (all - a.int_slot_count);
}
template <bool SPLIT, int KIND = 0>
__device__ __forceinline__ KsIdx ks_index(const KsMacArgs& a)
{
    const unsigned b = blockIdx.x, xcd = b & 7u, j = b >> 3;
    const unsigned splits = SPLIT ? (unsigned) a.splits : 1u;
    const unsigned units = (unsigned) a.items * splits;
    const unsigned tiles = 1u << (a.n_power - 12);
    const unsigned total = ks_slots(a, KIND) * tiles * units, chunk = (total + 7u) >> 3;
    const unsigned lin = xcd * chunk + j;
    const unsigned g = lin / units, unit = lin - g * units;
    const unsigned item = SPLIT ? unit / splits : unit, sp = SPLIT ? unit - item * splits : 0u;
    const unsigned nslots = ks_slots(a, KIND), gt = g / nslots;
    KsIdx r;
    r.valid = lin < total;
    r.item = (int) item;
    r.tile = (int) gt;
    int si = (int) (g - gt * nslots);
    if (KIND == 1 && a.int_slot_count > 0) {
        si = a.int_slots[r.valid ? si : 0];
    } else {
        si += a.slot_first;
        if (KIND == 2 && a.int_slot_count > 0) {
#pragma unroll
            for (int q = 0; q < 8; q++)
                if (q < a.int_slot_count && a.int_slots[q] <= si) si++;
        }
    }
    r.slot = si;
    r.d0 = SPLIT ? (int) (sp * (unsigned) a.digits / splits) : 0;
    r.d1 = SPLIT ? (int) ((sp + 1) * (unsigned) a.digits / splits) : a.digits;
    return r;
}

__device__ __forceinline__ void ks_tail_scatter(const KsMacArgs& a, int item, int slot, int p, u64 e0, const u64 (&r)[16])
{
    const KsMacArgs::Tail& e = a.tail;
    u64* out = e.out + e.out_item_stride * item + ((u64) (p * e.limbs + slot) << a.n_power);
    if (e.galois_inv) {
#pragma unroll
        for (int k = 0; k < 16; k++) {
            const u32 el = (u32) e0 + 16 * k;
            const u32 ex = ((2u * (__brev(el) >> (32 - a.n_power)) + 1u) * e.galois_inv) & ((2u << a.n_power) - 1u);
            out[__brev((ex - 1u) >> 1) >> (32 - a.n_power)] = r[k];
        }
    } else {
#pragma unroll
        for (int k = 0; k < 16; k++) out[e0 + 16 * k] = r[k];
    }
}
__device__ __forceinline__ void ks_tail_store(const KsMacArgs& a, int item, int slot, int p, u64 e0, const Mod& md, u64 inv,
                                              const u64 (&acc)[16], const u64 (&tv)[16], bool with_ct, const u64 (&cv)[16])
{
    u64 r[16];
#pragma unroll
    for (int k = 0; k < 16; k++) r[k] = mul_barrett(sub_mod(acc[k], tv[k], md.q), inv, md);
    if (with_ct) {
#pragma unroll
        for (int k = 0; k < 16; k++) r[k] = add_mod(cv[k], r[k], md.q);
    }
    ks_tail_scatter(a, item, slot, p, e0, r);
}
__device__ __forceinline__ void ks_tail_store_fp(const KsMacArgs& a, int item, int slot, int p, u64 e0, const FC& fc, double inv,
                                                 const double (&acc)[16], const double (&tv)[16], bool with_ct,
                                                 const u64 (&cv)[16])
{
    double m[16];
#pragma unroll
    for (int k = 0; k < 16; k++) {
        FP_STAGE(fc, FP_STAGE_OUT);
        const double d = fp_reduce(acc[k], fc) - tv[k];
        FP_STAGE(fc, FP_STAGE_TAIL);
        FP_AUDIT_VAL(fc, FPM_SUM, d);
        m[k] = fp_mul_nc(d, inv, fc);
    }
    FP_STAGE(fc, FP_STAGE_OUT);
    if (with_ct) {
#pragma unroll
        for (int k = 0; k < 16; k++) m[k] += fp_from_u64(cv[k]);
    }
    u64 r[16];
#pragma unroll
    for (int k = 0; k < 16; k++) r[k] = fp_to_u64(fp_canon(m[k], fc));
    ks_tail_scatter(a, item, slot, p, e0, r);
}
__device__ __forceinline__ const u64* ks_tail_T(const KsMacArgs& a, int item, int slot, int tile, int p)
{
    return a.tail.T + a.tail.T_item_stride * item + ((u64) (p * a.rc + slot) << a.n_power) + (u64) tile * 4096;
}
__device__ __forceinline__ bool ks_tail_ct(const KsMacArgs& a, int item, int slot, int p, u64 e0, u64 (&cv)[16])
{
    const KsMacArgs::Tail& e = a.tail;
    if (!e.ct || (e.ct_parts && p >= e.ct_parts)) return false;
    const u64* c = e.ct + e.ct_item_stride * item + ((u64) (p * e.limbs + slot) << a.n_power) + e0;
#pragma unroll
    for (int k = 0; k < 16; k++) cv[k] = c[16 * k];
    return true;
}

#define KS_TW_LDS_BYTES ((15 * 256 + 15 * 16) * 8)
template <bool SPLIT, bool MD = false>
__device__ __forceinline__ void ks_row_mac_int_body(const KsMacArgs& a, const KsIdx& ki, const Mod& md, int midx,
                                                    u64* lds, void* twbuf)
{
    const int t = threadIdx.x;
    const int item = ki.item, tile = ki.tile, slot = ki.slot;
    const QC qc = make_qc(md.q);
    const int s1 = a.n_power - 8;
    const ulonglong2* __restrict__ tw = a.tw + ((u64) midx << a.n_power);
    const int row = t >> 4, i0 = t & 15;
    const u32 crow = tile * 16 + row;
    const ulonglong2* __restrict__ tb = a.twB + ((u64) midx * (15u << (a.n_power - 4))) + ((u64) crow * 15 * 16 + i0);
    const u64 n = (u64) 1 << a.n_power;
    const u64* __restrict__ pin = a.in + a.in_item_stride * item + ((u64) slot << a.n_power) + (u64) tile * 4096;
    const u64* __restrict__ pk = a.key + ((u64) midx << a.n_power) + (u64) tile * 4096 + row * 256 + i0;
    const u64 dig_off = (u64) a.rc << a.n_power;
    const u64 key_off1 = (u64) a.key_limbs << a.n_power, key_off2 = (u64) a.key_limbs << (a.n_power + 1);
    const bool lazy = row_stages_lazy(md, a.lazy_q_max) && md.q <= ~0ull / (u64) a.digits;
    const bool room16 = stages_room16(md);
    const int ex = a.unreduced_exit;
    ulonglong2* twa = reinterpret_cast<ulonglong2*>(twbuf);
    if (i0 < 15) {
        const int s = (i0 >= 7) ? 3 : (i0 >= 3) ? 2 : (i0 >= 1) ? 1 : 0;
        twa[i0 * 16 + row] = tw[((((u32) 1 << s1) + crow) << s) + (i0 - ((1 << s) - 1))];
    }
    wave_lds_fence();

    const int item_s = MD ? __builtin_amdgcn_readfirstlane(item) : 0, slot_s = MD ? __builtin_amdgcn_readfirstlane(slot) : 0;
    const int tile_s = MD ? __builtin_amdgcn_readfirstlane(tile) : 0, midx_s = MD ? __builtin_amdgcn_readfirstlane(midx) : 0;
    u64 h0[16], l0[16], h1[16], l1[16];
#pragma unroll
    for (int k = 0; k < 16; k++) h0[k] = l0[k] = h1[k] = l1[k] = 0;
    for (int i = ki.d0; i < ki.d1; i++) {
        u64 x[16];
        const u64* p = pin + dig_off * i;
        if (a.skip_identity && i == midx) {
            const u64* pi = a.ident + a.ident_item_stride * item + ((u64) i << a.n_power) + (u64) tile * 4096;
#pragma unroll
            for (int k = 0; k < 16; k++) x[k] = gld(&pi[row * 256 + i0 + 16 * k]);
        } else if (lazy) {
            ks_row_digit<true>(x, p, lds, twa, tb, qc, md, row, i0);
        } else if (room16) {
            if (ex == 16) ks_row_digit<false, 16, 16>(x, p, lds, twa, tb, qc, md, row, i0);
            else if (ex == 12) ks_row_digit<false, 16, 12>(x, p, lds, twa, tb, qc, md, row, i0);
            else if (ex == 8) ks_row_digit<false, 16, 8>(x, p, lds, twa, tb, qc, md, row, i0);
            else ks_row_digit<false, 16>(x, p, lds, twa, tb, qc, md, row, i0);
        } else {
            if (ex) ks_row_digit<false, 8, 8>(x, p, lds, twa, tb, qc, md, row, i0);
            else ks_row_digit<false>(x, p, lds, twa, tb, qc, md, row, i0);
        }
        const u64* k0 = pk + key_off2 * i;
        const u64* k1 = k0 + key_off1;
#pragma unroll
        for (int k = 0; k < 16; k++) {
            acc128(h0[k], l0[k], x[k], k0[16 * k]);
            acc128(h1[k], l1[k], x[k], k1[16 * k]);
        }
    }
    if constexpr (MD) {
        u64 acc0[16], acc1[16];
#pragma unroll
        for (int k = 0; k < 16; k++) {
            acc0[k] = reduce128(h0[k], l0[k], md);
            acc1[k] = reduce128(h1[k], l1[k], md);
        }
        int tt = threadIdx.x;
        asm volatile("" : "+v"(tt));
        const int trow = tt >> 4, ti0 = tt & 15;
        const u64 e0 = (u64) tile_s * 4096 + trow * 256 + ti0;
        const u64 inv = a.tail.inv[midx_s];
        const bool lazy_t = row_stages_lazy(md, a.lazy_q_max);
        const ulonglong2* __restrict__ ttb = a.twB + ((u64) midx_s * (15u << (a.n_power - 4))) + ((u64) (tile_s * 16 + trow) * 15 * 16 + ti0);
        auto part = [&](int p, const u64 (&acc)[16]) {
            u64 cv[16], x[16];
            const bool with_ct = ks_tail_ct(a, item_s, slot_s, p, e0, cv);
            const u64* pT = ks_tail_T(a, item_s, slot_s, tile_s, p);
            if (lazy_t) {
                ks_row_digit<true>(x, pT, lds, twa, ttb, qc, md, trow, ti0);
#pragma unroll
                for (int k = 0; k < 16; k++) x[k] = reduce64(x[k], md);
            } else if (room16) {
                ks_row_digit<false, 16>(x, pT, lds, twa, ttb, qc, md, trow, ti0);
            } else {
                ks_row_digit<false>(x, pT, lds, twa, ttb, qc, md, trow, ti0);
            }
            ks_tail_store(a, item_s, slot_s, p, e0, md, inv, acc, x, with_ct, cv);
        };
        __builtin_amdgcn_sched_barrier(0);
        part(0, acc0);
        __builtin_amdgcn_sched_barrier(0);
        part(1, acc1);
        return;
    }
    u64* po = (SPLIT ? const_cast<u64*>(pin) + dig_off * ki.d0 - (u64) tile * 4096
                     : a.out + a.out_item_stride * item + ((u64) slot << a.n_power)) +
              (u64) tile * 4096 + row * 256 + i0;
#pragma unroll
    for (int k = 0; k < 16; k++) {
        po[16 * k] = reduce128(h0[k], l0[k], md);
        po[dig_off + 16 * k] = reduce128(h1[k], l1[k], md);
    }
    (void) n;
}

template <bool SPLIT>
__global__ __launch_bounds__(NTT_THREADS, SPLIT ? 2 : 1) void ks_row_mac(KsMacArgs a)
{
    __shared__ __attribute__((aligned(16))) u64 lds[ROW_LDS_ELEMS];
    __shared__ ulonglong2 twa[15 * 16];
    const KsIdx ki = ks_index<SPLIT, SPLIT ? 0 : 1>(a);
    if (!ki.valid) return;
    const int midx = a.mod_order ? a.mod_order[ki.slot] : ki.slot;
    const Mod md = a.mods[midx];
    if (md.fp) return;
    ks_row_mac_int_body<SPLIT>(a, ki, md, midx, lds, twa);
}

template <bool SPLIT>
__device__ __forceinline__ void ks_fp_row(double (&x)[16], const u64 (&xr)[16], const double* twl, u64* lds, const FC& fc,
                                          int s1, int row, int i0, int t)
{
    if constexpr (SPLIT) {
#pragma unroll
        for (int k = 0; k < 16; k++) x[k] = as_f64(xr[k]);
#pragma unroll
        for (int s = 0; s < 4; s++) {
            const int half = 8 >> s;
            FP_STAGE(fc, s1 + s);
#pragma unroll
            for (int b = 0; b < (1 << s); b++) {
                const double w = twl[15 * 256 + ((1 << s) - 1 + b) * 16 + row];
#pragma unroll
                for (int j = 0; j < half; j++) fp_ct_bfly(x[b * 2 * half + j], x[b * 2 * half + j + half], w, fc);
            }
        }
        FP_STAGE(fc, s1 + 4);
#pragma unroll
        for (int k = 0; k < 16; k++) x[k] = fp_reduce(x[k], fc);
#pragma unroll
        for (int k = 0; k < 16; k++) lds[row_phys(row * 256 + i0 + 16 * k)] = as_bits(x[k]);
        wave_lds_fence();
#pragma unroll
        for (int k = 0; k < 8; k++) {
            ulonglong2 v = *reinterpret_cast<const ulonglong2*>(&lds[row_phys(row * 256 + 16 * i0 + 2 * k)]);
            x[2 * k] = as_f64(v.x);
            x[2 * k + 1] = as_f64(v.y);
        }
#pragma unroll
        for (int s = 0; s < 4; s++) {
            const int half = 8 >> s;
            FP_STAGE(fc, s1 + 4 + s);
#pragma unroll
            for (int b = 0; b < (1 << s); b++) {
                const double w = twl[((1 << s) - 1 + b) * 256 + t];
#pragma unroll
                for (int j = 0; j < half; j++) fp_ct_bfly(x[b * 2 * half + j], x[b * 2 * half + j + half], w, fc);
            }
        }
    } else {
        int row_o = row, t_o = t;
        asm volatile("" : "+v"(row_o), "+v"(t_o));
        const double* twa = twl + 15 * 256 + row_o;
        const double* twb = twl + t_o;
        double wn[8], wc[8];
        wc[0] = twa[0];
        wn[0] = twa[16];
        wn[1] = twa[32];
        __builtin_amdgcn_sched_barrier(0);
#pragma unroll
        for (int k = 0; k < 16; k++) x[k] = as_f64(xr[k]);
#pragma unroll
        for (int s = 0; s < 4; s++) {
            const int half = 8 >> s;
            FP_STAGE(fc, s1 + s);
            if (s > 0) {
#pragma unroll
                for (int b = 0; b < (1 << s); b++) wc[b] = wn[b];
            }
            if (s < 3) {
                if (s > 0) {
#pragma unroll
                    for (int b = 0; b < (2 << s); b++) wn[b] = twa[((2 << s) - 1 + b) * 16];
                }
            } else {
                wn[0] = twb[0];
            }
            __builtin_amdgcn_sched_barrier(0);
#pragma unroll
            for (int b = 0; b < (1 << s); b++) {
                const double w = wc[b];
#pragma unroll
                for (int j = 0; j < half; j++) fp_ct_bfly(x[b * 2 * half + j], x[b * 2 * half + j + half], w, fc);
            }
        }
        FP_STAGE(fc, s1 + 4);
#pragma unroll
        for (int k = 0; k < 16; k++) x[k] = fp_reduce(x[k], fc);
#pragma unroll
        for (int k = 0; k < 16; k++) lds[row_phys(row * 256 + i0 + 16 * k)] = as_bits(x[k]);
        wave_lds_fence();
#pragma unroll
        for (int k = 0; k < 8; k++) {
            ulonglong2 v = *reinterpret_cast<const ulonglong2*>(&lds[row_phys(row * 256 + 16 * i0 + 2 * k)]);
            x[2 * k] = as_f64(v.x);
            x[2 * k + 1] = as_f64(v.y);
        }
#pragma unroll
        for (int s = 0; s < 4; s++) {
            const int half = 8 >> s;
            FP_STAGE(fc, s1 + 4 + s);
#pragma unroll
            for (int b = 0; b < (1 << s); b++) wc[b] = wn[b];
            if (s < 3) {
#pragma unroll
                for (int b = 0; b < (2 << s); b++) wn[b] = twb[((2 << s) - 1 + b) * 256];
            }
            __builtin_amdgcn_sched_barrier(0);
#pragma unroll
            for (int b = 0; b < (1 << s); b++) {
                const double w = wc[b];
#pragma unroll
                for (int j = 0; j < half; j++) fp_ct_bfly(x[b * 2 * half + j], x[b * 2 * half + j + half], w, fc);
            }
        }
    }
    wave_lds_fence();
#pragma unroll
    for (int k = 0; k < 8; k++)
        *reinterpret_cast<ulonglong2*>(&lds[row_phys(row * 256 + 16 * i0 + 2 * k)]) =
            make_ulonglong2(as_bits(x[2 * k]), as_bits(x[2 * k + 1]));
    wave_lds_fence();
#pragma unroll
    for (int k = 0; k < 16; k++) x[k] = as_f64(lds[row_phys(row * 256 + i0 + 16 * k)]);
    wave_lds_fence();
}

template <bool SPLIT, bool MD = false>
__device__ __forceinline__ void ks_row_mac_fp_body(const KsMacArgs& a, const KsIdx& ki, const Mod& md, int midx,
                                                   u64* lds, void* twbuf)
{
    const int t = threadIdx.x;
    const int item = ki.item, tile = ki.tile, slot = ki.slot;
    const FC fc = make_fc(md.q, FP_SITE(SPLIT ? FPS_KS_ROW_SPLIT : FPS_KS_ROW, a.n_power - 12));
    const int s1 = a.n_power - 8;
    const ulonglong2* __restrict__ tw = a.tw + ((u64) midx << a.n_power);
    const int row = t >> 4, i0 = t & 15;
    const u32 crow = tile * 16 + row;
    const double* __restrict__ tb8 = a.twB8 + ((u64) midx * (15u << (a.n_power - 4))) + ((u64) crow * 15 * 16 + i0);
    const u64* __restrict__ pin = a.in + a.in_item_stride * item + ((u64) slot << a.n_power) + (u64) tile * 4096;
    const u64* __restrict__ pk = a.key + ((u64) midx << a.n_power) + (u64) tile * 4096 + row * 256 + i0;
    const u64 dig_off = (u64) a.rc << a.n_power;
    const u64 key_off1 = (u64) a.key_limbs << a.n_power, key_off2 = (u64) a.key_limbs << (a.n_power + 1);

    double* twl = reinterpret_cast<double*>(twbuf);
#pragma unroll
    for (int k = 0; k < 15; k++) twl[k * 256 + t] = tb8[k * 16];
    if (i0 < 15) {
        const int s = (i0 >= 7) ? 3 : (i0 >= 3) ? 2 : (i0 >= 1) ? 1 : 0;
        const int b = i0 - ((1 << s) - 1);
        twl[15 * 256 + i0 * 16 + row] = as_f64(tw[((((u32) 1 << s1) + crow) << s) + b].x);
    }
    wave_lds_fence();

    const int item_s = MD ? __builtin_amdgcn_readfirstlane(item) : 0, slot_s = MD ? __builtin_amdgcn_readfirstlane(slot) : 0;
    const int tile_s = MD ? __builtin_amdgcn_readfirstlane(tile) : 0, midx_s = MD ? __builtin_amdgcn_readfirstlane(midx) : 0;
    double a0[16], a1[16];
#pragma unroll
    for (int k = 0; k < 16; k++) a0[k] = a1[k] = 0.0;
    int since = 0;
    for (int i = ki.d0; i < ki.d1; i++) {
        double x[16];
        const u64* p = pin + dig_off * i;
        const bool ident = a.skip_identity && i == midx;
        const u64* px = ident ? a.ident + a.ident_item_stride * item + ((u64) i << a.n_power) + (u64) tile * 4096 : p;
        u64 xr[16];
#pragma unroll
        for (int k = 0; k < 16; k++) {
            if constexpr (!SPLIT) xr[k] = __builtin_nontemporal_load(&px[row * 256 + i0 + 16 * k]);
            else xr[k] = px[row * 256 + i0 + 16 * k];
        }
        const u64* k0 = pk + key_off2 * i;
        const u64* k1 = k0 + key_off1;
        u64 kv0[16], kv1[16];
#pragma unroll
        for (int k = 0; k < 16; k++) {
            kv0[k] = k0[16 * k];
            kv1[k] = k1[16 * k];
        }
        if (ident) {
            FP_STAGE(fc, FP_STAGE_INPUT);
#pragma unroll
            for (int k = 0; k < 16; k++) x[k] = fp_reduce(fp_from_u64_ldexp(xr[k]), fc);
        } else {
            ks_fp_row<SPLIT>(x, xr, twl, lds, fc, s1, row, i0, t);
        }
#pragma unroll
        for (int k = 0; k < 16; k++) {
            FP_STAGE(fc, FP_STAGE_PRODUCT);
            a0[k] += fp_mul_nc(fp_from_u64_ldexp(kv0[k]), x[k], fc);
            a1[k] += fp_mul_nc(fp_from_u64_ldexp(kv1[k]), x[k], fc);
            FP_STAGE(fc, FP_STAGE_SUMS + since);
            FP_AUDIT_VAL(fc, FPM_SUM, a0[k]);
            FP_AUDIT_VAL(fc, FPM_SUM, a1[k]);
        }
        if (++since == 3) {
            since = 0;
            FP_STAGE(fc, FP_STAGE_SUMS + 3);
#pragma unroll
            for (int k = 0; k < 16; k++) {
                a0[k] = fp_reduce(a0[k], fc);
                a1[k] = fp_reduce(a1[k], fc);
            }
        }
    }
    if constexpr (MD) {
        int tt = threadIdx.x;
        asm volatile("" : "+v"(tt));
        const int trow = tt >> 4, ti0 = tt & 15;
        const u64 e0 = (u64) tile_s * 4096 + trow * 256 + ti0;
        const double inv = fp_from_u64(a.tail.inv[midx_s]);
        auto part = [&](int p, const double (&acc)[16]) {
            const u64* pT = ks_tail_T(a, item_s, slot_s, tile_s, p);
            u64 tr[16], cv[16];
#pragma unroll
            for (int k = 0; k < 16; k++) tr[k] = __builtin_nontemporal_load(&pT[trow * 256 + ti0 + 16 * k]);
            const bool with_ct = ks_tail_ct(a, item_s, slot_s, p, e0, cv);
            double x[16];
            ks_fp_row<false>(x, tr, twl, lds, fc, s1, trow, ti0, tt);
            ks_tail_store_fp(a, item_s, slot_s, p, e0, fc, inv, acc, x, with_ct, cv);
        };
        __builtin_amdgcn_sched_barrier(0);
        part(0, a0);
        __builtin_amdgcn_sched_barrier(0);
        part(1, a1);
        return;
    }
    u64* po = (SPLIT ? const_cast<u64*>(pin) + dig_off * ki.d0 - (u64) tile * 4096
                     : a.out + a.out_item_stride * item + ((u64) slot << a.n_power)) +
              (u64) tile * 4096 + row * 256 + i0;
    FP_STAGE(fc, FP_STAGE_OUT);
#pragma unroll
    for (int k = 0; k < 16; k++) {
        if constexpr (!SPLIT) {
            __builtin_nontemporal_store(fp_to_u64(fp_canon(a0[k], fc)), &po[16 * k]);
            __builtin_nontemporal_store(fp_to_u64(fp_canon(a1[k], fc)), &po[dig_off + 16 * k]);
        } else {
            po[16 * k] = fp_to_u64(fp_canon(a0[k], fc));
            po[dig_off + 16 * k] = fp_to_u64(fp_canon(a1[k], fc));
        }
    }
}

template <bool SPLIT>
__global__ __launch_bounds__(NTT_THREADS) void ks_row_mac_fp(KsMacArgs a)
{
    __shared__ __attribute__((aligned(16))) u64 lds[ROW_LDS_ELEMS];
    __shared__ double twl[15 * 256 + 15 * 16];
    const KsIdx ki = ks_index<SPLIT, SPLIT ? 0 : 2>(a);
    if (!ki.valid) return;
    const int midx = a.mod_order ? a.mod_order[ki.slot] : ki.slot;
    const Mod md = a.mods[midx];
    if (!md.fp) return;
    ks_row_mac_fp_body<SPLIT>(a, ki, md, midx, lds, twl);
}

__global__ __launch_bounds__(NTT_THREADS) void ks_row_mac_fp_moddown(KsMacArgs a)
{
    __shared__ __attribute__((aligned(16))) u64 lds[ROW_LDS_ELEMS];
    __shared__ double twl[15 * 256 + 15 * 16];
    const KsIdx ki = ks_index<false, 2>(a);
    if (!ki.valid) return;
    const int midx = a.mod_order ? a.mod_order[ki.slot] : ki.slot;
    const Mod md = a.mods[midx];
    if (!md.fp) return;
    ks_row_mac_fp_body<false, true>(a, ki, md, midx, lds, twl);
}
__global__ __launch_bounds__(NTT_THREADS, 1) void ks_row_mac_moddown(KsMacArgs a)
{
    __shared__ __attribute__((aligned(16))) u64 lds[ROW_LDS_ELEMS];
    __shared__ ulonglong2 twa[15 * 16];
    const KsIdx ki = ks_index<false, 1>(a);
    if (!ki.valid) return;
    const int midx = a.mod_order ? a.mod_order[ki.slot] : ki.slot;
    const Mod md = a.mods[midx];
    if (md.fp) return;
    ks_row_mac_int_body<false, true>(a, ki, md, midx, lds, twa);
}

__global__ __launch_bounds__(NTT_THREADS, 2) void ks_row_mac_split(KsMacArgs a)
{
    __shared__ __attribute__((aligned(16))) u64 lds[ROW_LDS_ELEMS];
    __shared__ double twl[15 * 256 + 15 * 16];
    const KsIdx ki = ks_index<true>(a);
    if (!ki.valid) return;
    const int midx = a.mod_order ? a.mod_order[ki.slot] : ki.slot;
    const Mod md = a.mods[midx];
    if (md.fp) ks_row_mac_fp_body<true>(a, ki, md, midx, lds, twl);
    else ks_row_mac_int_body<true>(a, ki, md, midx, lds, twl);
}

hipError_t ks_row_mac_launch(const KsMacArgs& a, int items, hipStream_t st)
{
    if (a.digits > 64 || items <= 0) return hipErrorInvalidValue;
    if (a.splits > 1 && a.digits < 2 * a.splits) return hipErrorInvalidValue;
    if (a.tail.on && (a.splits > 1 || !a.tail.out || !a.tail.T || !a.tail.inv)) return hipErrorInvalidValue;
    if (a.slot_first < 0 || a.slot_count < 0 || a.slot_first + (a.slot_count ? a.slot_count : a.rc) > a.rc)
        return hipErrorInvalidValue;
    KsMacArgs k = a;
    k.items = items;
    if (k.int_slot_count < 0 || k.int_slot_count > 8) k.int_slot_count = 0;
    const unsigned tiles = (1u << a.n_power) / 4096, units = (unsigned) items * (a.splits > 1 ? (unsigned) a.splits : 1u);
    auto grid_of = [&](int kind) { return dim3(8u * ((ks_slots(k, kind) * tiles * units + 7u) / 8u)); };
    if (a.splits > 1) {
        hipLaunchKernelGGL(ks_row_mac_split, grid_of(0), dim3(NTT_THREADS), 0, st, k);
    } else {
        if (!a.no_fp && ks_slots(k, 2) > 0) {
            if (a.tail.on) hipLaunchKernelGGL(ks_row_mac_fp_moddown, grid_of(2), dim3(NTT_THREADS), 0, st, k);
            else hipLaunchKernelGGL(ks_row_mac_fp<false>, grid_of(2), dim3(NTT_THREADS), 0, st, k);
        }
        if (!a.no_int && ks_slots(k, 1) > 0) {
            if (a.tail.on) hipLaunchKernelGGL(ks_row_mac_moddown, grid_of(1), dim3(NTT_THREADS), 0, st, k);
            else hipLaunchKernelGGL(ks_row_mac<false>, grid_of(1), dim3(NTT_THREADS), 0, st, k);
        }
    }
    return hipGetLastError();
}

__device__ __forceinline__ void fp_gs_bfly(double& x, double& y, ulonglong2 w, const FC& c)
{
    const double s = x + y, d = x - y;
    x = s;
    y = fp_mul(d, as_f64(w.x), as_f64(w.y), c);
    FP_AUDIT_VAL(c, FPM_SUM, s);
}

struct ArInt {
    typedef u64 T;
    QC qc;
    __device__ __forceinline__ explicit ArInt(const Mod& md) : qc(make_qc(md.q)) {}
    __device__ __forceinline__ T from_canon(u64 v) const { return v; }
    __device__ __forceinline__ T from_bits(u64 v) const { return v; }
    __device__ __forceinline__ u64 to_bits(T v) const { return v; }
    template <int LOGR>
    __device__ __forceinline__ void radix(T (&x)[1 << LOGR], const ulonglong2* __restrict__ tw, u32 root0) const
    {
        gs_radix<LOGR>(x, tw, root0, qc);
    }
    __device__ __forceinline__ void radix16_tb(T (&x)[16], const ulonglong2* __restrict__ tb) const { gs_radix16_tb(x, tb, qc); }
    template <int LOGR>
    __device__ __forceinline__ void radix_last(T (&x)[1 << LOGR], const ulonglong2* __restrict__ tw, ulonglong2 ninv,
                                               ulonglong2 w1ninv, u64 (&out)[1 << LOGR]) const
    {
        gs_radix_last<LOGR>(x, tw, 1u, ninv, w1ninv, qc);
#pragma unroll
        for (int k = 0; k < (1 << LOGR); k++) out[k] = x[k];
    }
};

struct ArFp {
    typedef double T;
    FC fc;
    int s1;
    __device__ __forceinline__ explicit ArFp(const Mod& md, int n_power) : fc(make_fc(md.q, FP_SITE(FPS_INV, n_power - 12))), s1(n_power - 8) {}
    __device__ __forceinline__ T from_canon(u64 v) const { return fp_from_u64(v); }
    __device__ __forceinline__ T from_bits(u64 v) const { return as_f64(v); }
    __device__ __forceinline__ u64 to_bits(T v) const { return as_bits(v); }
    template <int N>
    __device__ __forceinline__ void reduce_all(T (&x)[N]) const
    {
#pragma unroll
        for (int k = 0; k < N; k++) x[k] = fp_reduce(x[k], fc);
    }
    template <int LOGR>
    __device__ __forceinline__ void radix(T (&x)[1 << LOGR], const ulonglong2* __restrict__ tw, u32 root0) const
    {
        int done = 0;
#pragma unroll
        for (int s = LOGR - 1; s >= 0; s--) {
            const int half = (1 << LOGR) >> (s + 1);
            FP_STAGE(fc, 31 - __builtin_clz(root0) + s);
#pragma unroll
            for (int b = 0; b < (1 << s); b++) {
                const ulonglong2 w = tw[(root0 << s) + b];
#pragma unroll
                for (int j = 0; j < half; j++) fp_gs_bfly(x[b * 2 * half + j], x[b * 2 * half + j + half], w, fc);
            }
            if ((++done & 1) == 0 || s == 0) reduce_all(x);
        }
    }
    __device__ __forceinline__ void radix16_tb(T (&x)[16], const ulonglong2* __restrict__ tb) const
    {
#pragma unroll
        for (int s = 3; s >= 0; s--) {
            const int half = 8 >> s;
            FP_STAGE(fc, s1 + 4 + s);
#pragma unroll
            for (int b = 0; b < (1 << s); b++) {
                const ulonglong2 w = tb[((1 << s) - 1 + b) * 16];
#pragma unroll
                for (int j = 0; j < half; j++) fp_gs_bfly(x[b * 2 * half + j], x[b * 2 * half + j + half], w, fc);
            }
            if (s == 2 || s == 0) reduce_all(x);
        }
    }
    template <int LOGR>
    __device__ __forceinline__ void radix_last(T (&x)[1 << LOGR], const ulonglong2* __restrict__ tw, ulonglong2 ninv,
                                               ulonglong2 w1ninv, u64 (&out)[1 << LOGR]) const
    {
        int done = 0;
#pragma unroll
        for (int s = LOGR - 1; s >= 1; s--) {
            const int half = (1 << LOGR) >> (s + 1);
            FP_STAGE(fc, s);
#pragma unroll
            for (int b = 0; b < (1 << s); b++) {
                const ulonglong2 w = tw[(1u << s) + b];
#pragma unroll
                for (int j = 0; j < half; j++) fp_gs_bfly(x[b * 2 * half + j], x[b * 2 * half + j + half], w, fc);
            }
            if ((++done & 1) == 0) reduce_all(x);
        }
        constexpr int half = (1 << LOGR) >> 1;
        FP_STAGE(fc, 0);
#pragma unroll
        for (int j = 0; j < half; j++) {
            const double sum = x[j] + x[j + half], d = x[j] - x[j + half];
            out[j] = fp_to_u64(fp_canon(fp_mul(sum, as_f64(ninv.x), as_f64(ninv.y), fc), fc));
            out[j + half] = fp_to_u64(fp_canon(fp_mul(d, as_f64(w1ninv.x), as_f64(w1ninv.y), fc), fc));
        }
    }
};

template <typename AR, bool TO_LDS, bool TENSOR = false>
__device__ __forceinline__ void inv_row_part(const AR& ar, const NttArgs& a, int mod, int tt, u32 crow0,
                                             const u64* __restrict__ src, u64* __restrict__ dst, u64* lds,
                                             int tensor_part = 0)
{
    typedef typename AR::T T;
    const int s1 = a.n_power - 8;
    const ulonglong2* __restrict__ tw = a.itw + ((u64) mod << a.n_power);
    const int row = tt >> 4, i0 = tt & 15;
    const u32 crow = crow0 + row;
    if (TENSOR) {
        const Mod md = a.mods[mod];
        const u64 part_off = (u64) a.tensor_limbs << a.n_power;
        const u64* __restrict__ a0 = src, * __restrict__ a1 = src + part_off, * __restrict__ b0 = src + 2 * part_off,
                 * __restrict__ b1 = src + 3 * part_off;
#pragma unroll
        for (int k0 = 0; k0 < 16; k0 += 4) {
            u64 r[4];
            if (tensor_part == 1) {
                u64 va0[4], va1[4], vb0[4], vb1[4];
#pragma unroll
                for (int k = 0; k < 4; k++) {
                    const int e = row * 256 + i0 + 16 * (k0 + k);
                    va0[k] = a0[e]; va1[k] = a1[e]; vb0[k] = b0[e]; vb1[k] = b1[e];
                }
#pragma unroll
                for (int k = 0; k < 4; k++) {
                    u64 h1, l1, h2, l2;
                    mul64wide(va0[k], vb1[k], h1, l1);
                    mul64wide(va1[k], vb0[k], h2, l2);
                    const u64 lo = l1 + l2;
                    r[k] = reduce128(h1 + h2 + (lo < l1), lo, md);
                }
            } else {
                const u64* __restrict__ pa = tensor_part == 0 ? a0 : a1;
// ... 644 lines not shown
```

### heongpu_amd/csrc/ntt.hpp

```cpp
#pragma once
#include "modarith.cuh"

namespace hegpu {

struct NttEpilogue {
    const u64* ks;
    u64 ks_item_stride;
    int ks_part_limbs;
    const u64* ct;
    u64 ct_item_stride;
    int ct_parts;
    unsigned galois_inv;
    u64* out;
    u64 out_item_stride;
    const u64* inv;
    int limbs;
    int on;
    unsigned mg_limbs;
};

struct NttInvEpilogue {
    int on;
    int limbs;
    int add_parts;
    int p_mod;
    int galois_elt;
    unsigned mg_slots;
    u64 half;
    const u64* half_mod;
    const u64* inv;
    const u64* ct;
    u64 ct_item_stride;
    u64* out;
    u64 out_item_stride;
    int p_count;
    const u64* u;
    u64 u_item_stride;
};

struct NttArgs {
    const u64* in;
    u64* out;
    const Mod* mods;
    const ulonglong2* tw;
    const ulonglong2* itw;
    const ulonglong2* twB;
    const ulonglong2* itwB;
    const double* twB8;
    const ulonglong2* ninv;
    const ulonglong2* w1ninv;
    const int* mod_order;
    const int* poly_order;
    int n_power;
    int mod_count;
    int mod_offset;
    int polys_per_item;
    u64 in_item_stride;
    u64 out_item_stride;
    int decomp_mods;
    int skip_identity;
    int group_span;
    unsigned mg_group_span, mg_per_item, mg_polys_per_item, mg_mod_count, mg_decomp_mods;
    NttEpilogue epi;
    NttInvEpilogue iepi;
    int decomp_in_mul, decomp_in_add;
    int decomp_out_mul;
    int half_on, half_src_mod;
    u64 half;
    const u64* half_mod;
    int col_multi;
    int single_pass;
    int plan_has_fp, plan_has_int;
    u64 lazy_q_max;
    int only_int;
    int single_decomp_ok;
    int int_slot_count;
    int int_slots[8];
    int src_inv;
    const u64* copy_src;
    u64* copy_dst;
    u64 copy_src_item_stride, copy_dst_item_stride;
    int copy_part_limbs;
    const u64* tensor_in;
    u64 tensor_item_stride;
    int tensor_limbs;
    unsigned mg_tensor_limbs;
};

hipError_t ntt_launch(const NttArgs& a, int batch, bool inverse, hipStream_t st);
bool ntt_decomp_uses_multi(const NttArgs& a, int batch);
hipError_t ntt_launch_inv_rows(const NttArgs& a, int batch, hipStream_t st);
hipError_t ntt_launch_fwd_col(const NttArgs& a, int batch, hipStream_t st);

struct KsMacArgs {
    const u64* in;
    u64 in_item_stride;
    const u64* key;
    u64* out;
    u64 out_item_stride;
    const Mod* mods;
    const ulonglong2* tw;
    const ulonglong2* twB;
    const double* twB8;
    const int* mod_order;
    int n_power, digits, rc, key_limbs;
    u64 lazy_q_max;
    int skip_identity;
    const u64* ident;
    u64 ident_item_stride;
    int items;
    int splits;
    int no_fp, no_int;
    int int_slot_count;
    int int_slots[8];
    int slot_first, slot_count;
    int unreduced_exit;
    struct Tail {
        int on;
        const u64* T;
        u64 T_item_stride;
        const u64* ct;
        u64 ct_item_stride;
        int ct_parts;
        unsigned galois_inv;
        u64* out;
        u64 out_item_stride;
        const u64* inv;
        int limbs;
    } tail;
};
hipError_t ks_row_mac_launch(const KsMacArgs& a, int items, hipStream_t st);
constexpr inline int ks_unreduced_exit(int digits, int q_bits)
{
    if (digits <= 0 || q_bits <= 0 || 2 * q_bits > 127) return 0;
    const unsigned __int128 room = ((unsigned __int128) 1 << (128 - 2 * q_bits));
    for (int b = 16; b >= 8; b -= 4)
        if ((unsigned __int128) digits * (unsigned) b <= room) return b;
    return 0;
}

}
```

### heongpu_amd/csrc/ops.cpp

```cpp
#include "ops.hpp"
#include <algorithm>
#include <vector>
#include <utility>

namespace hegpu {

#define TRY(x)                           \
    do {                                 \
        hipError_t e__ = (x);            \
        if (e__ != hipSuccess) return e__; \
    } while (0)

static u64 inv_mod_2n(u64 g, u64 two_n)
{
    u64 x = g;
    for (int i = 0; i < 6; i++) x *= 2 - g * x;
    return x & (two_n - 1);
}

static long fused_row_mac_need(const Context& c)
{
    size_t fp = 0;
    for (unsigned char f : c.plan_qp.fp) fp += f ? 1 : 0;
    return (2 * fp > c.plan_qp.fp.size()) ? 768 : 400;
}
static int fused_digit_splits(const Context& c, int rc, int digits, int batch)
{
    if (c.digit_split == 0) return 0;
    if (c.digit_split > 0) return digits >= 2 * c.digit_split ? c.digit_split : 0;
    if (c.fused_row_mac >= 0 || c.n_power < 16 || digits < 8) return 0;
    const long wgs = (long) batch * rc * (long) (c.n >> 12), need = fused_row_mac_need(c);
    return (need == 768 && wgs < 2 * need && 4 * wgs >= need) ? 4 : 0;
}
static bool use_fused_row_mac(const Context& c, int rc, int batch)
{
    if (c.fused_row_mac >= 0) return c.fused_row_mac != 0;
    return (long) batch * rc * (long) (c.n >> 12) >= fused_row_mac_need(c);
}
static bool use_moddown_in_mac(const Context& c, const u64* key, int l, int rc, int batch)
{
    return c.moddown_in_mac && c.fused_moddown && key && c.P_size == 1 && use_fused_row_mac(c, rc, batch) &&
           !fused_digit_splits(c, rc, l, batch) && (long) 2 * l * batch <= 65535;
}

static void fill_int_slots(const Context& c, NttArgs& a, const u64* order)
{
    int cnt = 0;
    for (int k = 0; k < a.decomp_mods; k++) {
        const int m = a.mod_offset + (order ? (int) order[k] : k);
        if (m < 0 || m >= (int) c.plan_qp.fp.size()) { a.int_slot_count = 0; return; }
        if (c.plan_qp.fp[m]) continue;
        if (cnt == 8) { a.int_slot_count = 0; return; }
        a.int_slots[cnt++] = k;
    }
    a.int_slot_count = cnt ? cnt : -1;
}

static int launch_int_q_bits(const Context& c, const int* order, int rc, int depth, int slot_first, int slot_count)
{
    const NttPlan& p = c.plan_qp;
    const u64* ho = nullptr;
    const size_t off = (size_t) triangle_offset(c.Qp_size, depth);
    if (order && order == c.tab.new_prime_locations + off && off + (size_t) rc <= c.hv.new_prime_locations.size())
        ho = c.hv.new_prime_locations.data() + off;
    int bits = 0;
    auto take = [&](size_t m) { if (m < p.bits.size() && !p.fp[m] && p.bits[m] > bits) bits = p.bits[m]; };
    if (order && !ho) {
        for (size_t m = 0; m < p.bits.size(); m++) take(m);
        return bits;
    }
    const int k0 = slot_count ? slot_first : 0, k1 = slot_count ? slot_first + slot_count : rc;
    for (int k = k0; k < k1; k++) take(ho ? (size_t) ho[k] : (size_t) k);
    return bits;
}

static hipError_t keyswitch_ntt_mac(const Context& c, NttArgs a, const u64* key, u64* acc, u64 acc_stride,
                                    int digits, int rc, int split, int level, const u64* ident, u64 ident_stride,
                                    int batch, hipStream_t st, int which = 3, int slot_first = 0, int slot_count = 0,
                                    const KsMacArgs::Tail* tail = nullptr)
{
    const int ppi = digits * rc;
    const int skip_identity = ident ? 1 : 0;
    a.skip_identity = skip_identity;
    const int splits = fused_digit_splits(c, rc, digits, batch);
    if (!splits && !use_fused_row_mac(c, rc, batch)) {
        if (slot_count || tail) return hipErrorInvalidValue;
        if (ident && c.fused_row_mac == 0)
            TRY(rns_copy_diag(ident, ident_stride, a.out, a.out_item_stride, c.n_power, digits, rc, batch, st));
        else a.skip_identity = 0;
        TRY(ntt_launch(a, ppi * batch, false, st));
        return rns_keyswitch_mac(a.out, a.out_item_stride, key, acc, acc_stride, c.plan_qp.mods, c.n_power, digits, rc,
                                 c.Qp_size, split, level, batch, st);
    }
    const int chunk = 65535 / ppi;
    if (chunk < 1) return hipErrorInvalidValue;
    for (int b0 = 0; b0 < batch; b0 += chunk) {
        const int nb = (batch - b0 < chunk) ? batch - b0 : chunk;
        NttArgs ca = a;
        ca.in = a.in + (u64) b0 * a.in_item_stride;
        ca.out = a.out + (u64) b0 * a.out_item_stride;
        if (which & 1) TRY(ntt_launch_fwd_col(ca, ppi * nb, st));
        if (!(which & 2)) continue;
        KsMacArgs k{};
        k.in = ca.out; k.in_item_stride = a.out_item_stride; k.key = key;
        k.out = acc + (u64) b0 * acc_stride; k.out_item_stride = acc_stride;
        k.mods = c.plan_qp.mods; k.tw = c.plan_qp.tw; k.twB = c.plan_qp.twB; k.twB8 = c.plan_qp.twB8; k.mod_order = a.mod_order;
        k.lazy_q_max = a.lazy_q_max; k.n_power = c.n_power; k.digits = digits; k.rc = rc; k.key_limbs = c.Qp_size; k.skip_identity = skip_identity;
        k.ident = ident ? ident + (u64) b0 * ident_stride : nullptr; k.ident_item_stride = ident_stride;
        k.splits = splits;
        k.no_fp = !a.plan_has_fp;
        k.no_int = !a.plan_has_int || a.int_slot_count < 0;
        k.int_slot_count = a.int_slot_count > 0 ? a.int_slot_count : 0;
        for (int q = 0; q < 8; q++) k.int_slots[q] = a.int_slots[q];
        k.slot_first = slot_first; k.slot_count = slot_count;
        k.unreduced_exit = ks_unreduced_exit(splits > 1 ? (digits + splits - 1) / splits : digits,
                                             launch_int_q_bits(c, a.mod_order, rc, level, slot_first, slot_count));
        if (slot_count && a.int_slot_count > 0) {
            int cnt = 0;
            for (int q = 0; q < a.int_slot_count; q++)
                if (a.int_slots[q] >= slot_first && a.int_slots[q] < slot_first + slot_count) k.int_slots[cnt++] = a.int_slots[q];
            k.int_slot_count = cnt;
            k.no_int = cnt == 0;
            k.no_fp = k.no_fp || cnt == slot_count;
        }
        if (tail) {
            k.tail = *tail;
            k.tail.T += (u64) b0 * tail->T_item_stride;
            if (tail->ct) k.tail.ct += (u64) b0 * tail->ct_item_stride;
            k.tail.out += (u64) b0 * tail->out_item_stride;
        }
        TRY(ks_row_mac_launch(k, nb, st));
        if (splits > 1)
            TRY(rns_sum_partials(ca.out, a.out_item_stride, k.out, acc_stride, c.plan_qp.mods, a.mod_order, c.n_power,
                                 digits, rc, splits, nb, st));
    }
    return hipSuccess;
}


struct KeySwitchWs { u64 digits, acc, acc_words, per; };
static KeySwitchWs keyswitch_ws(const Context& c, int depth, bool copy, int accs)
{
    const u64 l = c.Q_size - depth, rc = c.Qp_size - depth;
    const u64 digits = copy ? 2 * l * c.n : 0, acc = digits + l * rc * c.n, acc_words = 2 * rc * c.n;
    return {digits, acc, acc_words, acc + accs * acc_words};
}
int ops_rotate_hoisted_accumulators(const Context& c, int depth, int batch, size_t ws_elems)
{
    return ws_elems >= keyswitch_ws(c, depth, true, 4).per * (u64) batch ? 4 : 1;
}

struct PairWs { u64 second, per; };
static PairWs rescale_ws(const Context& c, int depth)
{
    const u64 l = c.Q_size - depth;
    return {2 * (l - 1) * c.n, (2 * (l - 1) + 2 * l) * c.n};
}
static u64 mod_raise_ws(const Context& c) { return 2 * c.n; }
static PairWs bfv_multiply_ws(const Context& c)
{
    const u64 L = c.Q_size + c.bsk_size;
    return {4 * L * c.n, (4 + 3) * L * c.n};
}
static PairWs ckks_decode_ws(const Context& c, int depth) { const u64 l = c.Q_size - depth; return {l * c.n, (l + 1) * c.n}; }
static PairWs public_key_share_ws(const Context& c) { return {(u64) c.Qp_size * c.n, (u64) 2 * c.Qp_size * c.n}; }
static PairWs switch_key_share_ws(const Context& c, int errs)
{
    return {(u64) errs * switch_key_digits(c) * c.Qp_size * c.n, (u64) (errs + 1) * c.Q_size * c.Qp_size * c.n};
}
struct EncryptWs { u64 e, pku, per; };
static EncryptWs encrypt_ws(const Context& c)
{
    const u64 limb = (u64) c.Qp_size * c.n;
    return {limb, 3 * limb, 5 * limb};
}
struct RefreshMergeWs { u64 head_sum, total; };
static RefreshMergeWs bfv_refresh_merge_ws(const Context& c, int batch)
{
    return {(u64) batch * c.n, (u64) (c.Q_size + 1) * c.n * batch};
}
struct GateWs { u64 ps, ks, total; };
static GateWs gate_ws(const Context& c, bool bfv, int depth, int batch)
{
    const auto row = [&](int op) { return ops_workspace_elems(c, op, bfv ? 0 : depth, batch); };
    const size_t most = bfv ? std::max({row(OP_BFV_MULTIPLY), row(OP_BFV_RELIN), row(OP_BFV_MULTIPLY_PLAIN)})
                            : std::max(row(OP_CKKS_RELIN), row(OP_CKKS_RESCALE));
    const u64 ps = (u64) 3 * (bfv ? c.Q_size : c.Q_size - depth) * c.n, ks = ps * batch;
    return {ps, ks, ks + most};
}

size_t ops_workspace_elems(const Context& c, int op, int depth, int batch)
{
    const u64 n = c.n;
    u64 per = 0;
    switch (op) {
        case OP_CKKS_RELIN: per = keyswitch_ws(c, depth, false, 1).per; break;
        case OP_CKKS_RESCALE: per = rescale_ws(c, depth).per; break;
        case OP_CKKS_GALOIS: per = keyswitch_ws(c, depth, true, 1).per; break;
        case OP_CKKS_ROTATE_HOISTED: per = keyswitch_ws(c, depth, true, 4).per; break;
        case OP_BFV_MULTIPLY: per = bfv_multiply_ws(c).per; break;
        case OP_BFV_RELIN:
        case OP_BFV_GALOIS: per = keyswitch_ws(c, 0, false, 1).per; break;
        case OP_KEYGEN_SECRET: per = n; break;
        case OP_KEYGEN_PUBLIC: per = public_key_share_ws(c).per; break;
        case OP_KEYGEN_SWITCH: per = switch_key_share_ws(c, 1).per; break;
        case OP_CKKS_ENCRYPT:
        case OP_BFV_ENCRYPT: per = encrypt_ws(c).per; break;
        case OP_BFV_DECRYPT: per = (u64) c.Q_size * n; break;
        case OP_BFV_DECODE: per = n; break;
        case OP_BFV_MULTIPLY_PLAIN: per = (u64) c.Q_size * n; break;
        case OP_CKKS_ENCODE: per = n; break;
        case OP_CKKS_DECODE: per = ckks_decode_ws(c, depth).per; break;
        case OP_MPC_KEY_SHARE: per = switch_key_share_ws(c, 2).per; break;
        case OP_MPC_BFV_DECRYPT_MERGE: per = (u64) c.Q_size * n; break;
        case OP_MPC_REFRESH_SHARE: per = 0; break;
        case OP_MPC_REFRESH_MERGE:
            if (c.scheme != SCHEME_CKKS) return bfv_refresh_merge_ws(c, batch).total;
            per = (u64) (c.Q_size - depth) * n;
            break;
        case OP_CKKS_MOD_RAISE: per = mod_raise_ws(c); break;
        case OP_CKKS_BOOTSTRAP: per = 3 * mod_raise_ws(c); break;
        case OP_CKKS_LOGIC_GATE: return gate_ws(c, false, depth, batch).total;
        case OP_BFV_LOGIC_GATE: return gate_ws(c, true, depth, batch).total;
        default: return 0;
    }
    return per * (u64) batch;
}

hipError_t op_ckks_multiply(const Context& c, const u64* ct1, u64 s1, const u64* ct2, u64 s2, u64* out, u64 so,
                            int depth, int batch, hipStream_t st)
{
    if (batch <= 0) return hipSuccess;
    return rns_cross_multiplication(ct1, s1, ct2, s2, out, so, c.plan_qp.mods, c.n_power, c.Q_size - depth, batch,
                                    st);
}

static hipError_t ckks_keyswitch_core(const Context& c, const u64* src, u64 src_stride, const u64* add, u64 add_stride,
                                      int add_parts, u64* outp, u64 out_stride, const u64* key, int depth, int batch,
                                      u64* temp1, u64* temp2, u64 per, hipStream_t st, unsigned phases,
                                      int galois_elt = 0)
{
    const int Q = c.Q_size, Qp = c.Qp_size;
    const int l = Q - depth, rc = Qp - depth;

    NttArgs a = c.ntt_args(0);
    a.in = src; a.out = temp2; a.mod_count = l; a.polys_per_item = l;
    a.in_item_stride = src_stride; a.out_item_stride = per;
    NttArgs dgt = c.ntt_args(0);
    dgt.in = temp2; dgt.out = temp1; dgt.mod_count = rc; dgt.polys_per_item = l * rc; dgt.decomp_mods = rc;
    dgt.in_item_stride = per; dgt.out_item_stride = per;
    dgt.mod_order = c.tab.new_prime_locations + triangle_offset(Qp, depth);
    fill_int_slots(c, dgt, c.hv.new_prime_locations.data() + triangle_offset(Qp, depth));
    const bool fuse_inv = use_fused_row_mac(c, rc, batch) && c.fuse_inverse && (long) l * rc * batch <= 65535 &&
                          ntt_decomp_uses_multi(dgt, l * rc * batch);
    if (phases & RELIN_PHASE_INTT_C2) {
        if (fuse_inv) TRY(ntt_launch_inv_rows(a, l * batch, st));
        else TRY(ntt_launch(a, l * batch, true, st));
    }
    dgt.src_inv = fuse_inv ? 1 : 0;
    dgt.single_decomp_ok = 1;
    a = dgt;
    const int which = ((phases & RELIN_PHASE_COLUMN) ? 1 : 0) | ((phases & RELIN_PHASE_ROW_MAC) ? 2 : 0);
// ... 1334 lines not shown
```

### include/hegpu_bench.h

```cpp
#ifndef HEGPU_BENCH_H
#define HEGPU_BENCH_H
#include "hegpu.h"
#ifdef __cplusplus
extern "C" {
#endif
int hegpu_probe_ckks_relinearize(hegpu_context* ctx, uint64_t* ct, uint64_t ct_stride, const uint64_t* relin_key,
                                 int depth, int batch, void* ws, size_t ws_bytes, unsigned phases,
                                 hegpu_stream stream);
#ifdef __cplusplus
}
#endif
#endif
```

Baseline: 9004.

## Add paired 128-bit access variant of key-switch row MAC kernels

Adds a PAIR template mode to the key-switch row MAC kernels in which each thread owns adjacent element pairs rather than a stride-16 set. Key, input identity, tail ciphertext and output accesses then become 16-byte vector loads and stores, and the LDS readback uses an XOR-swizzled pair pattern. The mode is selected when pointers are 16-byte aligned and strides are even, is on by default through a new wide_access option, and launch-form counters are added for probing. It changes element-to-thread ownership, including the Galois scatter path, so any mismatch with other layout assumptions would risk incorrect results.

```diff
diff --git a/heongpu_amd/__init__.py b/heongpu_amd/__init__.py
--- a/heongpu_amd/__init__.py
+++ b/heongpu_amd/__init__.py
@@ -6,12 +6,12 @@
                   OP_CKKS_DECODE, OP_BFV_MULTIPLY_PLAIN, OP_MPC_KEY_SHARE, OP_MPC_BFV_DECRYPT_MERGE, OP_MPC_REFRESH_SHARE, OP_MPC_REFRESH_MERGE,
                   MPC_PUBLIC_KEY,
                   MPC_GALOIS_KEY, MPC_RELIN_ROUND1, GATE_NAND, GATE_AND, GATE_AND_FIRST_NOT,
-                  GATE_NOR, GATE_OR, GATE_XNOR, GATE_XOR, GATE_NOT, steps_to_galois_elt, linear_transform_plan, encoding_transform_factors, poly_eval_plan, eval_mod_plan, PolyEvalPlan, bootstrap_plan, BootstrapPlan, OP_CKKS_MOD_RAISE, OP_CKKS_BOOTSTRAP, MONOMIAL, CHEBYSHEV, POLY_POWER, POLY_LEAF, POLY_COMBINE, POLY_TAIL_NONE, POLY_TAIL_ONE, to_device, to_host, default_options, broadcast_key, broadcast_bytes, broadcast_path_name,
+                  GATE_NOR, GATE_OR, GATE_XNOR, GATE_XOR, GATE_NOT, steps_to_galois_elt, ks_launch_forms, linear_transform_plan, encoding_transform_factors, poly_eval_plan, eval_mod_plan, PolyEvalPlan, bootstrap_plan, BootstrapPlan, OP_CKKS_MOD_RAISE, OP_CKKS_BOOTSTRAP, MONOMIAL, CHEBYSHEV, POLY_POWER, POLY_LEAF, POLY_COMBINE, POLY_TAIL_NONE, POLY_TAIL_ONE, to_device, to_host, default_options, broadcast_key, broadcast_bytes, broadcast_path_name,
                   BCAST_FLAT, BCAST_TREE, BCAST_STAGED, BCAST_SAME_DEVICE, OP_CKKS_LOGIC_GATE, OP_BFV_LOGIC_GATE, LOGIC_AND,
                   LOGIC_OR, LOGIC_XOR, LOGIC_NAND, LOGIC_NOR, LOGIC_XNOR, LOGIC_NOT, GATE_B_NONE, GATE_B_CIPHER, GATE_B_PLAIN)
 
 _lib.load()
 
 __all__ = ["BFV", "CKKS", "SEC_NONE", "SEC_128", "SEC_192", "SEC_256", "TABLES_QP", "TABLES_Q_BSK", "Context", "HEError", "Rng",
-           "steps_to_galois_elt", "linear_transform_plan", "encoding_transform_factors", "poly_eval_plan", "eval_mod_plan", "PolyEvalPlan", "bootstrap_plan", "BootstrapPlan", "MONOMIAL", "CHEBYSHEV", "POLY_POWER", "POLY_LEAF", "POLY_COMBINE", "POLY_TAIL_NONE", "POLY_TAIL_ONE", "to_device", "to_host", "default_options", "broadcast_key", "broadcast_bytes", "broadcast_path_name",
+           "steps_to_galois_elt", "ks_launch_forms", "linear_transform_plan", "encoding_transform_factors", "poly_eval_plan", "eval_mod_plan", "PolyEvalPlan", "bootstrap_plan", "BootstrapPlan", "MONOMIAL", "CHEBYSHEV", "POLY_POWER", "POLY_LEAF", "POLY_COMBINE", "POLY_TAIL_NONE", "POLY_TAIL_ONE", "to_device", "to_host", "default_options", "broadcast_key", "broadcast_bytes", "broadcast_path_name",
            "BCAST_FLAT", "BCAST_TREE", "BCAST_STAGED", "BCAST_SAME_DEVICE"]
diff --git a/heongpu_amd/_lib.py b/heongpu_amd/_lib.py
--- a/heongpu_amd/_lib.py
+++ b/heongpu_amd/_lib.py
@@ -106,6 +106,7 @@
     ("hegpu_ckks_relinearize_inplace", c_int, [voidp, u64p, u64, u64p, c_int, c_int, voidp, c_size_t, voidp]),
     ("hegpu_probe_ckks_relinearize", c_int,
      [voidp, u64p, u64, u64p, c_int, c_int, voidp, c_size_t, ctypes.c_uint, voidp]),
+    ("hegpu_probe_ks_launch_forms", None, [u64p]),
     ("hegpu_ckks_rescale_inplace", c_int, [voidp, u64p, u64, c_int, c_int, voidp, c_size_t, voidp]),
     ("hegpu_ckks_apply_galois", c_int,
      [voidp, u64p, u64, u64p, u64, u64p, c_int, c_int, c_int, voidp, c_size_t, voidp]),
diff --git a/heongpu_amd/api.py b/heongpu_amd/api.py
--- a/heongpu_amd/api.py
+++ b/heongpu_amd/api.py
@@ -1077,5 +1077,11 @@
                                           c.eval_target_scale, pr))
 
 
+def ks_launch_forms():
+    c = (ctypes.c_uint64 * 3)()
+    _lib.load().hegpu_probe_ks_launch_forms(c)
+    return tuple(int(x) for x in c)
+
+
 def steps_to_galois_elt(steps, n, group_order):
     return int(_lib.load().hegpu_steps_to_galois_elt(steps, n, group_order))
diff --git a/heongpu_amd/csrc/cabi.cpp b/heongpu_amd/csrc/cabi.cpp
--- a/heongpu_amd/csrc/cabi.cpp
+++ b/heongpu_amd/csrc/cabi.cpp
@@ -886,6 +886,13 @@
     return hip_ret(op_ckks_relinearize(ctx->c, (u64*) ct, cs, (const u64*) key, depth, batch, (u64*) ws,
                                        (hipStream_t) stream, phases),
                    "hegpu_probe_ckks_relinearize");
+}
+
+void hegpu_probe_ks_launch_forms(uint64_t counts[3])
+{
+    unsigned long long c[3];
+    ks_row_mac_launch_counts(c);
+    for (int i = 0; i < 3; i++) counts[i] = c[i];
 }
 
 int hegpu_ckks_rescale_inplace(hegpu_context* ctx, uint64_t* ct, uint64_t cs, int depth, int batch, void* ws,
diff --git a/heongpu_amd/csrc/context.cpp b/heongpu_amd/csrc/context.cpp
--- a/heongpu_amd/csrc/context.cpp
+++ b/heongpu_amd/csrc/context.cpp
@@ -718,6 +718,7 @@
     {"behz_split", "HEGPU_BEHZ_SPLIT", -1, 1, &H::behz_split, OptDesc::MIRROR_BEHZ},
     {"fused_tensor", "HEGPU_FUSED_TENSOR", &H::fused_tensor},
     {"moddown_in_mac", "HEGPU_MODDOWN_IN_MAC", &H::moddown_in_mac},
+    {"wide_access", "HEGPU_WIDE_ACCESS", &H::wide_access},
 };
 const OptDesc* find_option(const char* name)
 {
diff --git a/heongpu_amd/csrc/context.hpp b/heongpu_amd/csrc/context.hpp
--- a/heongpu_amd/csrc/context.hpp
+++ b/heongpu_amd/csrc/context.hpp
@@ -85,6 +85,7 @@
     bool copy_along = true;
     bool fuse_inverse = true;
     bool moddown_in_mac = true;
+    bool wide_access = true;
     bool fused_tensor = true;
     bool fp_ntt = true;
     int behz_split = -1;
diff --git a/heongpu_amd/csrc/ntt.hip b/heongpu_amd/csrc/ntt.hip
--- a/heongpu_amd/csrc/ntt.hip
+++ b/heongpu_amd/csrc/ntt.hip
@@ -1,4 +1,5 @@
 #include "ntt.hpp"
+#include <atomic>
 #define HEGPU_FP_TU ntt
 #include "fpmod.cuh"
 
@@ -941,7 +942,64 @@
 static_assert(ks_unreduced_exit(22, 60) == 8 && ks_unreduced_exit(32, 60) == 8 && ks_unreduced_exit(33, 60) == 0, "");
 static_assert(ks_unreduced_exit(4, 61) == 16 && ks_unreduced_exit(8, 61) == 8 && ks_unreduced_exit(9, 61) == 0, "");
 
-template <bool LAZY, int ROOM = 8, int EXIT = 0>
+template <bool PAIR> __device__ __forceinline__ int ks_own0(int i0) { return PAIR ? 2 * i0 : i0; }
+template <bool PAIR> __device__ __forceinline__ constexpr int ks_own(int k) { return PAIR ? 32 * (k >> 1) + (k & 1) : 16 * k; }
+template <bool PAIR, bool NT = false>
+__device__ __forceinline__ void ks_ld16(u64 (&v)[16], const u64* p)
+{
+    if constexpr (PAIR) {
+#pragma unroll
+        for (int m = 0; m < 8; m++) {
+            const u64x2_t* q = reinterpret_cast<const u64x2_t*>(p + 32 * m);
+            const u64x2_t w = NT ? __builtin_nontemporal_load(q) : *q;
+            v[2 * m] = w.x;
+            v[2 * m + 1] = w.y;
+        }
+    } else {
+#pragma unroll
+        for (int k = 0; k < 16; k++) v[k] = NT ? __builtin_nontemporal_load(&p[16 * k]) : p[16 * k];
+    }
+}
+template <bool PAIR, bool NT = false>
+__device__ __forceinline__ void ks_st16(u64* p, const u64 (&v)[16])
+{
+    if constexpr (PAIR) {
+#pragma unroll
+        for (int m = 0; m < 8; m++) {
+            u64x2_t w;
+            w.x = v[2 * m];
+            w.y = v[2 * m + 1];
+            u64x2_t* q = reinterpret_cast<u64x2_t*>(p + 32 * m);
+            if constexpr (NT) __builtin_nontemporal_store(w, q);
+            else *q = w;
+        }
+    } else {
+#pragma unroll
+        for (int k = 0; k < 16; k++) {
+            if constexpr (NT) __builtin_nontemporal_store(v[k], &p[16 * k]);
+            else p[16 * k] = v[k];
+        }
+    }
+}
+template <bool PAIR>
+__device__ __forceinline__ void ks_own_read(u64 (&v)[16], const u64* lds, int row, int i0)
+{
+    if constexpr (PAIR) {
+        int b = row * 256 + 2 * i0;
+        asm volatile("" : "+v"(b));
+#pragma unroll
+        for (int m = 0; m < 8; m++) {
+            const ulonglong2 w = *reinterpret_cast<const ulonglong2*>(&lds[(b ^ (2 * m)) + 32 * m]);
+            v[2 * m] = w.x;
+            v[2 * m + 1] = w.y;
+        }
+    } else {
+#pragma unroll
+        for (int k = 0; k < 16; k++) v[k] = lds[row_phys(row * 256 + i0 + 16 * k)];
+    }
+}
+
+template <bool LAZY, int ROOM = 8, int EXIT = 0, bool PAIR = false>
 __device__ __forceinline__ void ks_row_digit(u64 (&x)[16], const u64* __restrict__ p, u64* lds,
                                              const ulonglong2* twa, const ulonglong2* __restrict__ tb,
                                              const QC& qc, const Mod& md, int row, int i0)
@@ -981,8 +1039,7 @@
         *reinterpret_cast<ulonglong2*>(&lds[row_phys(row * 256 + 16 * i0 + 2 * k)]) =
             make_ulonglong2(x[2 * k], x[2 * k + 1]);
     wave_lds_fence();
-#pragma unroll
-    for (int k = 0; k < 16; k++) x[k] = lds[row_phys(row * 256 + i0 + 16 * k)];
+    ks_own_read<PAIR>(x, lds, row, i0);
     wave_lds_fence();
 }
 
@@ -1026,6 +1083,7 @@
     return r;
 }
 
+template <bool PAIR = false>
 __device__ __forceinline__ void ks_tail_scatter(const KsMacArgs& a, int item, int slot, int p, u64 e0, const u64 (&r)[16])
 {
     const KsMacArgs::Tail& e = a.tail;
@@ -1033,15 +1091,15 @@
     if (e.galois_inv) {
 #pragma unroll
         for (int k = 0; k < 16; k++) {
-            const u32 el = (u32) e0 + 16 * k;
+            const u32 el = (u32) e0 + ks_own<PAIR>(k);
             const u32 ex = ((2u * (__brev(el) >> (32 - a.n_power)) + 1u) * e.galois_inv) & ((2u << a.n_power) - 1u);
             out[__brev((ex - 1u) >> 1) >> (32 - a.n_power)] = r[k];
         }
     } else {
-#pragma unroll
-        for (int k = 0; k < 16; k++) out[e0 + 16 * k] = r[k];
-    }
-}
+        ks_st16<PAIR>(out + e0, r);
+    }
+}
+template <bool PAIR = false>
 __device__ __forceinline__ void ks_tail_store(const KsMacArgs& a, int item, int slot, int p, u64 e0, const Mod& md, u64 inv,
                                               const u64 (&acc)[16], const u64 (&tv)[16], bool with_ct, const u64 (&cv)[16])
 {
@@ -1052,8 +1110,9 @@
 #pragma unroll
         for (int k = 0; k < 16; k++) r[k] = add_mod(cv[k], r[k], md.q);
     }
-    ks_tail_scatter(a, item, slot, p, e0, r);
-}
+    ks_tail_scatter<PAIR>(a, item, slot, p, e0, r);
+}
+template <bool PAIR = false>
 __device__ __forceinline__ void ks_tail_store_fp(const KsMacArgs& a, int item, int slot, int p, u64 e0, const FC& fc, double inv,
                                                  const double (&acc)[16], const double (&tv)[16], bool with_ct,
                                                  const u64 (&cv)[16])
@@ -1075,24 +1134,24 @@
     u64 r[16];
 #pragma unroll
     for (int k = 0; k < 16; k++) r[k] = fp_to_u64(fp_canon(m[k], fc));
-    ks_tail_scatter(a, item, slot, p, e0, r);
+    ks_tail_scatter<PAIR>(a, item, slot, p, e0, r);
 }
 __device__ __forceinline__ const u64* ks_tail_T(const KsMacArgs& a, int item, int slot, int tile, int p)
 {
     return a.tail.T + a.tail.T_item_stride * item + ((u64) (p * a.rc + slot) << a.n_power) + (u64) tile * 4096;
 }
+template <bool PAIR = false>
 __device__ __forceinline__ bool ks_tail_ct(const KsMacArgs& a, int item, int slot, int p, u64 e0, u64 (&cv)[16])
 {
     const KsMacArgs::Tail& e = a.tail;
     if (!e.ct || (e.ct_parts && p >= e.ct_parts)) return false;
     const u64* c = e.ct + e.ct_item_stride * item + ((u64) (p * e.limbs + slot) << a.n_power) + e0;
-#pragma unroll
-    for (int k = 0; k < 16; k++) cv[k] = c[16 * k];
+    ks_ld16<PAIR>(cv, c);
     return true;
 }
 
 #define KS_TW_LDS_BYTES ((15 * 256 + 15 * 16) * 8)
-template <bool SPLIT, bool MD = false>
+template <bool SPLIT, bool MD = false, bool PAIR = false>
 __device__ __forceinline__ void ks_row_mac_int_body(const KsMacArgs& a, const KsIdx& ki, const Mod& md, int midx,
                                                     u64* lds, void* twbuf)
 {
@@ -1106,7 +1165,7 @@
     const ulonglong2* __restrict__ tb = a.twB + ((u64) midx * (15u << (a.n_power - 4))) + ((u64) crow * 15 * 16 + i0);
     const u64 n = (u64) 1 << a.n_power;
     const u64* __restrict__ pin = a.in + a.in_item_stride * item + ((u64) slot << a.n_power) + (u64) tile * 4096;
-    const u64* __restrict__ pk = a.key + ((u64) midx << a.n_power) + (u64) tile * 4096 + row * 256 + i0;
+    const u64* __restrict__ pk = a.key + ((u64) midx << a.n_power) + (u64) tile * 4096 + row * 256 + ks_own0<PAIR>(i0);
     const u64 dig_off = (u64) a.rc << a.n_power;
     const u64 key_off1 = (u64) a.key_limbs << a.n_power, key_off2 = (u64) a.key_limbs << (a.n_power + 1);
     const bool lazy = row_stages_lazy(md, a.lazy_q_max) && md.q <= ~0ull / (u64) a.digits;
@@ -1129,25 +1188,41 @@
         const u64* p = pin + dig_off * i;
         if (a.skip_identity && i == midx) {
             const u64* pi = a.ident + a.ident_item_stride * item + ((u64) i << a.n_power) + (u64) tile * 4096;
-#pragma unroll
-            for (int k = 0; k < 16; k++) x[k] = gld(&pi[row * 256 + i0 + 16 * k]);
+            if constexpr (PAIR) {
+                ks_ld16<true>(x, pi + row * 256 + 2 * i0);
+            } else {
+#pragma unroll
+                for (int k = 0; k < 16; k++) x[k] = gld(&pi[row * 256 + i0 + 16 * k]);
+            }
         } else if (lazy) {
-            ks_row_digit<true>(x, p, lds, twa, tb, qc, md, row, i0);
+            ks_row_digit<true, 8, 0, PAIR>(x, p, lds, twa, tb, qc, md, row, i0);
         } else if (room16) {
-            if (ex == 16) ks_row_digit<false, 16, 16>(x, p, lds, twa, tb, qc, md, row, i0);
-            else if (ex == 12) ks_row_digit<false, 16, 12>(x, p, lds, twa, tb, qc, md, row, i0);
-            else if (ex == 8) ks_row_digit<false, 16, 8>(x, p, lds, twa, tb, qc, md, row, i0);
-            else ks_row_digit<false, 16>(x, p, lds, twa, tb, qc, md, row, i0);
+            if (ex == 16) ks_row_digit<false, 16, 16, PAIR>(x, p, lds, twa, tb, qc, md, row, i0);
+            else if (ex == 12) ks_row_digit<false, 16, 12, PAIR>(x, p, lds, twa, tb, qc, md, row, i0);
+            else if (ex == 8) ks_row_digit<false, 16, 8, PAIR>(x, p, lds, twa, tb, qc, md, row, i0);
+            else ks_row_digit<false, 16, 0, PAIR>(x, p, lds, twa, tb, qc, md, row, i0);
         } else {
-            if (ex) ks_row_digit<false, 8, 8>(x, p, lds, twa, tb, qc, md, row, i0);
-            else ks_row_digit<false>(x, p, lds, twa, tb, qc, md, row, i0);
+            if (ex) ks_row_digit<false, 8, 8, PAIR>(x, p, lds, twa, tb, qc, md, row, i0);
+            else ks_row_digit<false, 8, 0, PAIR>(x, p, lds, twa, tb, qc, md, row, i0);
         }
         const u64* k0 = pk + key_off2 * i;
         const u64* k1 = k0 + key_off1;
-#pragma unroll
-        for (int k = 0; k < 16; k++) {
-            acc128(h0[k], l0[k], x[k], k0[16 * k]);
-            acc128(h1[k], l1[k], x[k], k1[16 * k]);
+        if constexpr (PAIR) {
+#pragma unroll
+            for (int m = 0; m < 8; m++) {
+                const ulonglong2 v0 = *reinterpret_cast<const ulonglong2*>(k0 + 32 * m);
+                const ulonglong2 v1 = *reinterpret_cast<const ulonglong2*>(k1 + 32 * m);
+                acc128(h0[2 * m], l0[2 * m], x[2 * m], v0.x);
+                acc128(h1[2 * m], l1[2 * m], x[2 * m], v1.x);
+                acc128(h0[2 * m + 1], l0[2 * m + 1], x[2 * m + 1], v0.y);
+                acc128(h1[2 * m + 1], l1[2 * m + 1], x[2 * m + 1], v1.y);
+            }
+        } else {
+#pragma unroll
+            for (int k = 0; k < 16; k++) {
+                acc128(h0[k], l0[k], x[k], k0[16 * k]);
+                acc128(h1[k], l1[k], x[k], k1[16 * k]);
+            }
         }
     }
     if constexpr (MD) {
@@ -1160,24 +1235,24 @@
         int tt = threadIdx.x;
         asm volatile("" : "+v"(tt));
         const int trow = tt >> 4, ti0 = tt & 15;
-        const u64 e0 = (u64) tile_s * 4096 + trow * 256 + ti0;
+        const u64 e0 = (u64) tile_s * 4096 + trow * 256 + ks_own0<PAIR>(ti0);
         const u64 inv = a.tail.inv[midx_s];
         const bool lazy_t = row_stages_lazy(md, a.lazy_q_max);
         const ulonglong2* __restrict__ ttb = a.twB + ((u64) midx_s * (15u << (a.n_power - 4))) + ((u64) (tile_s * 16 + trow) * 15 * 16 + ti0);
         auto part = [&](int p, const u64 (&acc)[16]) {
             u64 cv[16], x[16];
-            const bool with_ct = ks_tail_ct(a, item_s, slot_s, p, e0, cv);
+            const bool with_ct = ks_tail_ct<PAIR>(a, item_s, slot_s, p, e0, cv);
             const u64* pT = ks_tail_T(a, item_s, slot_s, tile_s, p);
             if (lazy_t) {
-                ks_row_digit<true>(x, pT, lds, twa, ttb, qc, md, trow, ti0);
+                ks_row_digit<true, 8, 0, PAIR>(x, pT, lds, twa, ttb, qc, md, trow, ti0);
 #pragma unroll
                 for (int k = 0; k < 16; k++) x[k] = reduce64(x[k], md);
             } else if (room16) {
-                ks_row_digit<false, 16>(x, pT, lds, twa, ttb, qc, md, trow, ti0);
+                ks_row_digit<false, 16, 0, PAIR>(x, pT, lds, twa, ttb, qc, md, trow, ti0);
             } else {
-                ks_row_digit<false>(x, pT, lds, twa, ttb, qc, md, trow, ti0);
-            }
-            ks_tail_store(a, item_s, slot_s, p, e0, md, inv, acc, x, with_ct, cv);
+                ks_row_digit<false, 8, 0, PAIR>(x, pT, lds, twa, ttb, qc, md, trow, ti0);
+            }
+            ks_tail_store<PAIR>(a, item_s, slot_s, p, e0, md, inv, acc, x, with_ct, cv);
         };
         __builtin_amdgcn_sched_barrier(0);
         part(0, acc0);
@@ -1185,13 +1260,26 @@
         part(1, acc1);
         return;
     }
-    u64* po = (SPLIT ? const_cast<u64*>(pin) + dig_off * ki.d0 - (u64) tile * 4096
-                     : a.out + a.out_item_stride * item + ((u64) slot << a.n_power)) +
-              (u64) tile * 4096 + row * 256 + i0;
-#pragma unroll
-    for (int k = 0; k < 16; k++) {
-        po[16 * k] = reduce128(h0[k], l0[k], md);
-        po[dig_off + 16 * k] = reduce128(h1[k], l1[k], md);
+    if constexpr (PAIR) {
+        int tt = threadIdx.x;
+        asm volatile("" : "+v"(tt));
+        u64* pw = a.out + a.out_item_stride * item + ((u64) slot << a.n_power) + (u64) tile * 4096 + (tt >> 4) * 256 + 2 * (tt & 15);
+#pragma unroll
+        for (int m = 0; m < 8; m++) {
+            *reinterpret_cast<ulonglong2*>(pw + 32 * m) =
+                make_ulonglong2(reduce128(h0[2 * m], l0[2 * m], md), reduce128(h0[2 * m + 1], l0[2 * m + 1], md));
+            *reinterpret_cast<ulonglong2*>(pw + dig_off + 32 * m) =
+                make_ulonglong2(reduce128(h1[2 * m], l1[2 * m], md), reduce128(h1[2 * m + 1], l1[2 * m + 1], md));
+        }
+    } else {
+        u64* po = (SPLIT ? const_cast<u64*>(pin) + dig_off * ki.d0 - (u64) tile * 4096
+                         : a.out + a.out_item_stride * item + ((u64) slot << a.n_power)) +
+                  (u64) tile * 4096 + row * 256 + i0;
+#pragma unroll
+        for (int k = 0; k < 16; k++) {
+            po[16 * k] = reduce128(h0[k], l0[k], md);
+            po[dig_off + 16 * k] = reduce128(h1[k], l1[k], md);
+        }
     }
     (void) n;
 }
@@ -1209,7 +1297,7 @@
     ks_row_mac_int_body<SPLIT>(a, ki, md, midx, lds, twa);
 }
 
-template <bool SPLIT>
+template <bool SPLIT, bool PAIR = false>
 __device__ __forceinline__ void ks_fp_row(double (&x)[16], const u64 (&xr)[16], const double* twl, u64* lds, const FC& fc,
                                           int s1, int row, int i0, int t)
 {
@@ -1323,12 +1411,19 @@
         *reinterpret_cast<ulonglong2*>(&lds[row_phys(row * 256 + 16 * i0 + 2 * k)]) =
             make_ulonglong2(as_bits(x[2 * k]), as_bits(x[2 * k + 1]));
     wave_lds_fence();
-#pragma unroll
-    for (int k = 0; k < 16; k++) x[k] = as_f64(lds[row_phys(row * 256 + i0 + 16 * k)]);
+    if constexpr (PAIR) {
+        u64 xb[16];
+        ks_own_read<true>(xb, lds, row, i0);
+#pragma unroll
+        for (int k = 0; k < 16; k++) x[k] = as_f64(xb[k]);
+    } else {
+#pragma unroll
+        for (int k = 0; k < 16; k++) x[k] = as_f64(lds[row_phys(row * 256 + i0 + 16 * k)]);
+    }
     wave_lds_fence();
 }
 
-template <bool SPLIT, bool MD = false>
+template <bool SPLIT, bool MD = false, bool PAIR = false>
 __device__ __forceinline__ void ks_row_mac_fp_body(const KsMacArgs& a, const KsIdx& ki, const Mod& md, int midx,
                                                    u64* lds, void* twbuf)
 {
@@ -1341,7 +1436,7 @@
     const u32 crow = tile * 16 + row;
     const double* __restrict__ tb8 = a.twB8 + ((u64) midx * (15u << (a.n_power - 4))) + ((u64) crow * 15 * 16 + i0);
     const u64* __restrict__ pin = a.in + a.in_item_stride * item + ((u64) slot << a.n_power) + (u64) tile * 4096;
-    const u64* __restrict__ pk = a.key + ((u64) midx << a.n_power) + (u64) tile * 4096 + row * 256 + i0;
+    const u64* __restrict__ pk = a.key + ((u64) midx << a.n_power) + (u64) tile * 4096 + row * 256 + ks_own0<PAIR>(i0);
     const u64 dig_off = (u64) a.rc << a.n_power;
     const u64 key_off1 = (u64) a.key_limbs << a.n_power, key_off2 = (u64) a.key_limbs << (a.n_power + 1);
 
@@ -1367,25 +1462,41 @@
         const bool ident = a.skip_identity && i == midx;
         const u64* px = ident ? a.ident + a.ident_item_stride * item + ((u64) i << a.n_power) + (u64) tile * 4096 : p;
         u64 xr[16];
-#pragma unroll
-        for (int k = 0; k < 16; k++) {
-            if constexpr (!SPLIT) xr[k] = __builtin_nontemporal_load(&px[row * 256 + i0 + 16 * k]);
-            else xr[k] = px[row * 256 + i0 + 16 * k];
+        if (PAIR && ident) {
+            ks_ld16<PAIR, true>(xr, px + row * 256 + 2 * i0);
+        } else {
+#pragma unroll
+            for (int k = 0; k < 16; k++) {
+                if constexpr (!SPLIT) xr[k] = __builtin_nontemporal_load(&px[row * 256 + i0 + 16 * k]);
+                else xr[k] = px[row * 256 + i0 + 16 * k];
+            }
         }
         const u64* k0 = pk + key_off2 * i;
         const u64* k1 = k0 + key_off1;
         u64 kv0[16], kv1[16];
-#pragma unroll
-        for (int k = 0; k < 16; k++) {
-            kv0[k] = k0[16 * k];
-            kv1[k] = k1[16 * k];
+        if constexpr (PAIR) {
+#pragma unroll
+            for (int m = 0; m < 8; m++) {
+                const ulonglong2 v0 = *reinterpret_cast<const ulonglong2*>(k0 + 32 * m);
+                const ulonglong2 v1 = *reinterpret_cast<const ulonglong2*>(k1 + 32 * m);
+                kv0[2 * m] = v0.x;
+                kv0[2 * m + 1] = v0.y;
+                kv1[2 * m] = v1.x;
+                kv1[2 * m + 1] = v1.y;
+            }
+        } else {
+#pragma unroll
+            for (int k = 0; k < 16; k++) {
+                kv0[k] = k0[16 * k];
+                kv1[k] = k1[16 * k];
+            }
         }
         if (ident) {
             FP_STAGE(fc, FP_STAGE_INPUT);
 #pragma unroll
             for (int k = 0; k < 16; k++) x[k] = fp_reduce(fp_from_u64_ldexp(xr[k]), fc);
         } else {
-            ks_fp_row<SPLIT>(x, xr, twl, lds, fc, s1, row, i0, t);
+            ks_fp_row<SPLIT, PAIR>(x, xr, twl, lds, fc, s1, row, i0, t);
         }
 #pragma unroll
         for (int k = 0; k < 16; k++) {
@@ -1410,17 +1521,17 @@
         int tt = threadIdx.x;
         asm volatile("" : "+v"(tt));
         const int trow = tt >> 4, ti0 = tt & 15;
-        const u64 e0 = (u64) tile_s * 4096 + trow * 256 + ti0;
+        const u64 e0 = (u64) tile_s * 4096 + trow * 256 + ks_own0<PAIR>(ti0);
         const double inv = fp_from_u64(a.tail.inv[midx_s]);
         auto part = [&](int p, const double (&acc)[16]) {
             const u64* pT = ks_tail_T(a, item_s, slot_s, tile_s, p);
             u64 tr[16], cv[16];
 #pragma unroll
             for (int k = 0; k < 16; k++) tr[k] = __builtin_nontemporal_load(&pT[trow * 256 + ti0 + 16 * k]);
-            const bool with_ct = ks_tail_ct(a, item_s, slot_s, p, e0, cv);
+            const bool with_ct = ks_tail_ct<PAIR>(a, item_s, slot_s, p, e0, cv);
             double x[16];
-            ks_fp_row<false>(x, tr, twl, lds, fc, s1, trow, ti0, tt);
-            ks_tail_store_fp(a, item_s, slot_s, p, e0, fc, inv, acc, x, with_ct, cv);
+            ks_fp_row<false, PAIR>(x, tr, twl, lds, fc, s1, trow, ti0, tt);
+            ks_tail_store_fp<PAIR>(a, item_s, slot_s, p, e0, fc, inv, acc, x, with_ct, cv);
         };
         __builtin_amdgcn_sched_barrier(0);
         part(0, a0);
@@ -1430,8 +1541,19 @@
     }
     u64* po = (SPLIT ? const_cast<u64*>(pin) + dig_off * ki.d0 - (u64) tile * 4096
                      : a.out + a.out_item_stride * item + ((u64) slot << a.n_power)) +
-              (u64) tile * 4096 + row * 256 + i0;
+              (u64) tile * 4096 + row * 256 + ks_own0<PAIR>(i0);
     FP_STAGE(fc, FP_STAGE_OUT);
+    if constexpr (PAIR) {
+        u64 r0[16], r1[16];
+#pragma unroll
+        for (int k = 0; k < 16; k++) {
+            r0[k] = fp_to_u64(fp_canon(a0[k], fc));
+            r1[k] = fp_to_u64(fp_canon(a1[k], fc));
+        }
+        ks_st16<true, !SPLIT>(po, r0);
+        ks_st16<true, !SPLIT>(po + dig_off, r1);
+        return;
+    }
 #pragma unroll
     for (int k = 0; k < 16; k++) {
         if constexpr (!SPLIT) {
@@ -1480,6 +1602,31 @@
     ks_row_mac_int_body<false, true>(a, ki, md, midx, lds, twa);
 }
 
+template <bool MD>
+__global__ __launch_bounds__(NTT_THREADS, 2) void ks_pair_mac_fp(KsMacArgs a)
+{
+    __shared__ __attribute__((aligned(16))) u64 lds[ROW_LDS_ELEMS];
+    __shared__ double twl[15 * 256 + 15 * 16];
+    const KsIdx ki = ks_index<false, 2>(a);
+    if (!ki.valid) return;
+    const int midx = a.mod_order ? a.mod_order[ki.slot] : ki.slot;
+    const Mod md = a.mods[midx];
+    if (!md.fp) return;
+    ks_row_mac_fp_body<false, MD, true>(a, ki, md, midx, lds, twl);
+}
+template <bool MD>
+__global__ __launch_bounds__(NTT_THREADS, 2) void ks_pair_mac(KsMacArgs a)
+{
+    __shared__ __attribute__((aligned(16))) u64 lds[ROW_LDS_ELEMS];
+    __shared__ ulonglong2 twa[15 * 16];
+    const KsIdx ki = ks_index<false, 1>(a);
+    if (!ki.valid) return;
+    const int midx = a.mod_order ? a.mod_order[ki.slot] : ki.slot;
+    const Mod md = a.mods[midx];
+    if (md.fp) return;
+    ks_row_mac_int_body<false, MD, true>(a, ki, md, midx, lds, twa);
+}
+
 __global__ __launch_bounds__(NTT_THREADS, 2) void ks_row_mac_split(KsMacArgs a)
 {
     __shared__ __attribute__((aligned(16))) u64 lds[ROW_LDS_ELEMS];
@@ -1490,6 +1637,12 @@
     const Mod md = a.mods[midx];
     if (md.fp) ks_row_mac_fp_body<true>(a, ki, md, midx, lds, twl);
     else ks_row_mac_int_body<true>(a, ki, md, midx, lds, twl);
+}
+
+static std::atomic<unsigned long long> g_ks_forms[3];
+void ks_row_mac_launch_counts(unsigned long long out[3])
+{
+    for (int i = 0; i < 3; i++) out[i] = g_ks_forms[i].load(std::memory_order_relaxed);
 }
 
 hipError_t ks_row_mac_launch(const KsMacArgs& a, int items, hipStream_t st)
@@ -1504,8 +1657,23 @@
     if (k.int_slot_count < 0 || k.int_slot_count > 8) k.int_slot_count = 0;
     const unsigned tiles = (1u << a.n_power) / 4096, units = (unsigned) items * (a.splits > 1 ? (unsigned) a.splits : 1u);
     auto grid_of = [&](int kind) { return dim3(8u * ((ks_slots(k, kind) * tiles * units + 7u) / 8u)); };
+    auto pair_ok = [](const void* p, u64 stride) { return !(reinterpret_cast<uintptr_t>(p) & 15u) && !(stride & 1u); };
+    const bool wide = a.wide && a.splits <= 1 && pair_ok(a.key, 0) &&
+                      (a.tail.on ? pair_ok(a.tail.out, a.tail.out_item_stride) && pair_ok(a.tail.ct, a.tail.ct_item_stride)
+                                 : pair_ok(a.out, a.out_item_stride)) &&
+                      (!a.skip_identity || pair_ok(a.ident, a.ident_item_stride));
+    g_ks_forms[a.splits > 1 ? 2 : wide ? 1 : 0].fetch_add(1, std::memory_order_relaxed);
     if (a.splits > 1) {
         hipLaunchKernelGGL(ks_row_mac_split, grid_of(0), dim3(NTT_THREADS), 0, st, k);
+    } else if (wide) {
+        if (!a.no_fp && ks_slots(k, 2) > 0) {
+            if (a.tail.on) hipLaunchKernelGGL(ks_pair_mac_fp<true>, grid_of(2), dim3(NTT_THREADS), 0, st, k);
+            else hipLaunchKernelGGL(ks_pair_mac_fp<false>, grid_of(2), dim3(NTT_THREADS), 0, st, k);
+        }
+        if (!a.no_int && ks_slots(k, 1) > 0) {
+            if (a.tail.on) hipLaunchKernelGGL(ks_pair_mac<true>, grid_of(1), dim3(NTT_THREADS), 0, st, k);
+            else hipLaunchKernelGGL(ks_pair_mac<false>, grid_of(1), dim3(NTT_THREADS), 0, st, k);
+        }
     } else {
         if (!a.no_fp && ks_slots(k, 2) > 0) {
             if (a.tail.on) hipLaunchKernelGGL(ks_row_mac_fp_moddown, grid_of(2), dim3(NTT_THREADS), 0, st, k);
diff --git a/heongpu_amd/csrc/ntt.hpp b/heongpu_amd/csrc/ntt.hpp
--- a/heongpu_amd/csrc/ntt.hpp
+++ b/heongpu_amd/csrc/ntt.hpp
@@ -115,6 +115,7 @@
     int int_slots[8];
     int slot_first, slot_count;
     int unreduced_exit;
+    int wide;
     struct Tail {
         int on;
         const u64* T;
@@ -130,6 +131,7 @@
     } tail;
 };
 hipError_t ks_row_mac_launch(const KsMacArgs& a, int items, hipStream_t st);
+void ks_row_mac_launch_counts(unsigned long long out[3]);
 constexpr inline int ks_unreduced_exit(int digits, int q_bits)
 {
     if (digits <= 0 || q_bits <= 0 || 2 * q_bits > 127) return 0;
diff --git a/heongpu_amd/csrc/ops.cpp b/heongpu_amd/csrc/ops.cpp
--- a/heongpu_amd/csrc/ops.cpp
+++ b/heongpu_amd/csrc/ops.cpp
@@ -108,6 +108,7 @@
         k.lazy_q_max = a.lazy_q_max; k.n_power = c.n_power; k.digits = digits; k.rc = rc; k.key_limbs = c.Qp_size; k.skip_identity = skip_identity;
         k.ident = ident ? ident + (u64) b0 * ident_stride : nullptr; k.ident_item_stride = ident_stride;
         k.splits = splits;
+        k.wide = c.wide_access && splits <= 1;
         k.no_fp = !a.plan_has_fp;
         k.no_int = !a.plan_has_int || a.int_slot_count < 0;
         k.int_slot_count = a.int_slot_count > 0 ? a.int_slot_count : 0;
diff --git a/include/hegpu_bench.h b/include/hegpu_bench.h
--- a/include/hegpu_bench.h
+++ b/include/hegpu_bench.h
@@ -7,6 +7,7 @@
 int hegpu_probe_ckks_relinearize(hegpu_context* ctx, uint64_t* ct, uint64_t ct_stride, const uint64_t* relin_key,
                                  int depth, int batch, void* ws, size_t ws_bytes, unsigned phases,
                                  hegpu_stream stream);
+void hegpu_probe_ks_launch_forms(uint64_t counts[3]);
 #ifdef __cplusplus
 }
 #endif
```

Result: faster. 9141 (median of 6 runs) (+1.5%).
